# PixelClear/OclPathTracer

Measured on AMD Instinct MI355X. Metric: Msamples/sec (pixels x spp / s), cornellbox.bin 1024x1024, higher is better.
Workload: dtype f32; 1 GPU; BASELINE configs[2]: cornellbox.bin 1024x1024, 256 spp, depth 16, full path; render_lanes=2, checkpointed_launches=True, staging_ring_bytes=402653184, workspace_bytes=490036560

## Files before the change

### include/pt_shim.h

```cpp
#ifndef PT_SHIM_H
#define PT_SHIM_H

#include <stddef.h>
#include <stdint.h>

#ifdef __cplusplus
extern "C" {
#endif

#define PT_SHIM_ABI_VERSION 2

enum pt_status {
    PT_OK = 0,
    PT_ERR_INVALID = 1,
    PT_ERR_NO_DEVICE = 2,
    PT_ERR_OOM = 3,
    PT_ERR_HIP = 4,
    PT_ERR_NOT_FOUND = 5,
    PT_ERR_ARGS = 6,
    PT_ERR_RANGE = 7,
    PT_ERR_TRAVERSAL = 8
};

typedef struct pt_device_s* pt_device_t;
typedef struct pt_buffer_s* pt_buffer_t;
typedef struct pt_kernel_s* pt_kernel_t;
typedef struct pt_event_s* pt_event_t;

const char* pt_last_error(void);
int pt_abi_version(void);

int pt_init(void);
void pt_quit(void);
int pt_device_count(void);
int pt_device_create(int device_idx, pt_device_t* out);
int pt_device_destroy(pt_device_t dev);

enum pt_info_kind {
    PT_INFO_NAME = 0,
    PT_INFO_BOARD = 1,
    PT_INFO_VENDOR = 2,
    PT_INFO_VERSION = 3
};
int pt_device_info(pt_device_t dev, int kind, char out[128]);
uint64_t pt_device_max_alloc(pt_device_t dev);
uint64_t pt_device_mem_size(pt_device_t dev);
uint64_t pt_device_used_memory(pt_device_t dev);
uint64_t pt_device_peak_memory(pt_device_t dev);
uint64_t pt_device_workspace_memory(pt_device_t dev);
int pt_device_reserve_staging(pt_device_t dev, size_t bytes);
int pt_device_num_cus(pt_device_t dev);

#define PT_STREAM_LEGACY ((void*)1)
int pt_device_set_stream(pt_device_t dev, void* hip_stream);
void* pt_device_get_stream(pt_device_t dev);
int pt_device_wait_stream(pt_device_t dev, void* hip_stream);
int pt_device_wait_hip_event(pt_device_t dev, void* hip_event);
int pt_event_wait_on(pt_event_t ev, void* hip_stream);

int pt_sync(pt_device_t dev);
int pt_flush(pt_device_t dev);

enum pt_option {
    PT_OPT_BATCH_FRAMES = 0,
    PT_OPT_CHUNK_FRAMES = 1,
    PT_OPT_PROFILE_RETURN_TIME = 2,
    PT_OPT_RESERVED_3 = 3,
    PT_OPT_QUAD_FILTER = 4,
    PT_OPT_ACCEL = 5,
    PT_OPT_BVH_TALLY = 6,
    PT_OPT_PRIMARY_MASKS = 7,
    PT_OPT_BVH_STACK_LIMIT = 8,
    PT_OPT_RENDER_LANES = 9,
    PT_OPT_CHECKPOINT = 10,
    PT_OPT_BVH_BUILD_COUNT = 11
};
int pt_device_set_option(pt_device_t dev, int option, int64_t value);
int64_t pt_device_get_option(pt_device_t dev, int option);

int pt_buffer_alloc(pt_device_t dev, size_t bytes, pt_buffer_t* out);
int pt_buffer_wrap(pt_device_t dev, void* device_ptr, size_t bytes, pt_buffer_t* out);
int pt_buffer_free(pt_buffer_t buf);
size_t pt_buffer_size(pt_buffer_t buf);
void* pt_buffer_device_ptr(pt_buffer_t buf);
void* pt_buffer_address(pt_buffer_t buf);
int pt_buffer_write(pt_buffer_t dst, const void* host_src, size_t bytes, size_t dst_offset, pt_event_t ev);
int pt_buffer_read(pt_buffer_t src, void* host_dst, size_t bytes, size_t src_offset, pt_event_t ev);
int pt_buffer_copy(pt_buffer_t dst, pt_buffer_t src, size_t bytes, size_t dst_offset, size_t src_offset, pt_event_t ev);
void* pt_buffer_map(pt_buffer_t buf, size_t bytes, int blocking);
int pt_buffer_unmap(pt_buffer_t buf, void* host_ptr);

int pt_host_alloc(size_t bytes, void** out);
int pt_host_free(void* host_ptr);

int pt_event_create(pt_device_t dev, pt_event_t* out);
int pt_event_destroy(pt_event_t ev);
int pt_event_wait(pt_event_t ev);
int pt_event_is_complete(pt_event_t ev);
int pt_event_elapsed_ns(pt_event_t ev, uint64_t* ns_out);

int pt_kernel_get(pt_device_t dev, const char* file_name, const char* func_name, pt_kernel_t* out);

#define PT_MAX_ARG_SIZE 64
#define PT_MAX_ARG_COUNT 64

typedef struct pt_launch_arg {
    int32_t is_buffer;
    int32_t read_only;
    uint64_t size;
    pt_buffer_t buffer;
    unsigned char data[PT_MAX_ARG_SIZE];
} pt_launch_arg;

int pt_launch_2d(pt_device_t dev, pt_kernel_t kernel, const pt_launch_arg* args, int nargs,
                 int num_threads_x, int num_threads_y, int local_x, int local_y,
                 pt_event_t ev, float* ms_out);

typedef struct pt_render_params {
    int32_t width, height;
    int32_t frame_begin;
    int32_t frame_count;
    int32_t max_bounces;
    int32_t num_triangles;
    int32_t num_materials;
    int32_t stripe_rows;
    int32_t n_ranks;
    int32_t rank;
    int32_t reserved[6];
} pt_render_params;

int pt_local_rows(int height, int stripe_rows, int n_ranks, int rank);

enum {
    PT_STAT_SAMPLES = 0, PT_STAT_RAYS = 1,
    PT_STAT_BVH_NODES = 2, PT_STAT_BVH_TRIS = 3, PT_STAT_BVH_STEPS = 4 , PT_STAT_BVH_TRI_STEPS = 5,
    PT_STAT_BVH_MAX_STACK = 6 ,
    PT_STAT_CARRIED = 7 ,
    PT_STAT_BVH_GRAZING = 8,
    PT_STAT_WORDS = 16
};

int pt_render_frames(pt_device_t dev, pt_buffer_t triangles, pt_buffer_t materials,
                     pt_buffer_t framebuffer, const pt_render_params* params,
                     pt_buffer_t stats ,
                     pt_event_t ev);

typedef struct pt_camera {
    float eye[3];
    float center[3];
    float up[3];
    float fov_y_deg;
    int32_t reserved[6];
} pt_camera;

void pt_camera_reference(pt_camera* out);
int pt_camera_derive(const pt_camera* cam, float out[16]);
int pt_render_frames_camera(pt_device_t dev, pt_buffer_t triangles, pt_buffer_t materials, pt_buffer_t framebuffer,
                            const pt_render_params* params, const pt_camera* cam,
// ... 102 lines not shown
                       pt_buffer_t noise , pt_buffer_t summary , pt_event_t ev);

typedef struct pt_adaptive_rule {
    double tol2;
    double floor2;
    uint32_t min_samples;
    uint32_t max_samples;
    uint32_t reserved[2];
} pt_adaptive_rule;
typedef struct pt_pixel_slot { uint32_t pixel; uint32_t frame; } pt_pixel_slot;
size_t pt_adaptive_list_bytes(uint32_t num_pixels);
int pt_adaptive_select(pt_device_t dev, pt_buffer_t moments , uint32_t num_pixels,
                       const pt_adaptive_rule* rule, pt_buffer_t list , pt_event_t ev);
int pt_render_indirect_pixels(pt_device_t dev, pt_buffer_t triangles, pt_buffer_t materials,
                              pt_buffer_t lights , int mis,
                              pt_buffer_t light_counts ,
                              pt_buffer_t cdf, pt_buffer_t tri_q , pt_buffer_t samples ,
                              pt_buffer_t framebuffer, pt_buffer_t list, uint32_t num_listed, const pt_indirect_params* params,
                              const pt_roulette* roulette, const pt_camera* cam , pt_event_t ev);
int pt_sample_moments_pixels(pt_device_t dev, pt_buffer_t samples ,
                             pt_buffer_t moments , pt_buffer_t list, uint32_t num_listed, int32_t frame_count,
                             pt_event_t ev);

typedef struct pt_ris {
    int32_t candidates;
    int32_t reserved[3];
} pt_ris;
int pt_render_direct_ris(pt_device_t dev, pt_buffer_t triangles, pt_buffer_t materials,
                         pt_buffer_t lights , pt_buffer_t cdf, pt_buffer_t tri_q ,
                         pt_buffer_t samples , pt_buffer_t framebuffer, const pt_direct_params* params, const pt_ris* ris,
                         const pt_camera* cam , pt_event_t ev);
int pt_render_indirect_ris(pt_device_t dev, pt_buffer_t triangles, pt_buffer_t materials,
                           pt_buffer_t lights , int mis,
                           pt_buffer_t light_counts ,
                           pt_buffer_t cdf, pt_buffer_t tri_q , pt_buffer_t samples ,
                           pt_buffer_t framebuffer, const pt_indirect_params* params, const pt_roulette* roulette, const pt_ris* ris,
                           const pt_camera* cam , pt_event_t ev);
int pt_render_indirect_pixels_ris(pt_device_t dev, pt_buffer_t triangles, pt_buffer_t materials,
                                  pt_buffer_t lights , int mis,
                                  pt_buffer_t light_counts ,
                                  pt_buffer_t cdf, pt_buffer_t tri_q , pt_buffer_t samples ,
                                  pt_buffer_t framebuffer, pt_buffer_t list, uint32_t num_listed, const pt_indirect_params* params,
                                  const pt_roulette* roulette, const pt_ris* ris, const pt_camera* cam ,
                                  pt_event_t ev);

typedef struct pt_environment {
    int32_t size;
    int32_t env_samples;
    int32_t reserved[2];
} pt_environment;
size_t pt_env_table_bytes(int size);
int pt_env_table(pt_device_t dev, pt_buffer_t env , int size, pt_buffer_t cdf ,
                 pt_event_t ev);
int pt_render_direct_env(pt_device_t dev, pt_buffer_t triangles, pt_buffer_t materials,
                         pt_buffer_t lights , pt_buffer_t cdf, pt_buffer_t tri_q ,
                         pt_buffer_t env, pt_buffer_t env_cdf , pt_buffer_t samples ,
                         pt_buffer_t framebuffer, const pt_direct_params* params, const pt_environment* environment,
                         const pt_camera* cam , pt_event_t ev);
int pt_render_indirect_env(pt_device_t dev, pt_buffer_t triangles, pt_buffer_t materials,
                           pt_buffer_t lights ,
                           pt_buffer_t light_counts, pt_buffer_t cdf, pt_buffer_t tri_q ,
                           pt_buffer_t env, pt_buffer_t env_cdf , pt_buffer_t samples ,
                           pt_buffer_t framebuffer, const pt_indirect_params* params, const pt_roulette* roulette,
                           const pt_environment* environment, const pt_camera* cam , pt_event_t ev);

enum { PT_PROF_TRACE = 0, PT_PROF_FOLD = 1, PT_PROF_KINDS = 2 };
int pt_profile_enable(pt_device_t dev, int on);
int pt_profile_query(pt_device_t dev, int kind, double* total_ms, uint64_t* launches);
int pt_profile_query_union(pt_device_t dev, int kind, double* union_ms);
int pt_profile_reset(pt_device_t dev);

#define PT_BVH_SNAPSHOT_BIG_MAX 64
typedef struct pt_bvh_info {
    uint32_t records;
    int32_t num_big;
    int32_t num_triangles;
    float grid_min[3], grid_step[3];
    int32_t reserved[7];
} pt_bvh_info;
int pt_bvh_snapshot(pt_device_t dev, pt_bvh_info* info, void* records, size_t record_capacity, int32_t* big_indices);

int pt_primary_mask_snapshot(pt_device_t dev, uint32_t* num_pixels, void* masks, size_t capacity);

int pt_assemble_stripes(pt_device_t dev, pt_buffer_t gathered, pt_buffer_t image, int width,
                        int height, int stripe_rows, int n_ranks, int slab_rows, pt_event_t ev);

int pt_assemble_stripes_on(pt_device_t dev, pt_buffer_t gathered, pt_buffer_t image, int width, int height,
                           int stripe_rows, int n_ranks, int slab_rows, void* hip_stream);

int pt_tonemap_ppm(pt_device_t dev, pt_buffer_t framebuffer, pt_buffer_t rgb_i32, size_t num_pixels,
                   pt_event_t ev);

#ifdef __cplusplus
}
#endif
#endif
```

### oclpathtracer_amd/csrc/pt_kernels.h

```cpp
#pragma once

#include <hip/hip_runtime.h>
#include <stdint.h>

struct PtRawTriangle { float p1[4], p2[4], p3[4]; int32_t id; char pad[12]; };
struct PtRawMaterial { float albedo[4], emissive[4]; float roughness; int32_t type; char pad[24]; };
static_assert(sizeof(PtRawTriangle) == 64 && sizeof(PtRawMaterial) == 64, "record layout");

struct PtPrepTriangle {
    float p1[3];
    float e1[3];
    float e2[3];
    float pad0[3];
    float n[3];
    int32_t id;
};
static_assert(sizeof(PtPrepTriangle) == 64, "prep layout");

struct PtBvhNode {
    float lmin[3]; uint32_t link_l;
    float lmax[3]; uint32_t link_r;
    float rmin[3]; uint32_t pad0;
    float rmax[3]; uint32_t pad1;
};
static_assert(sizeof(PtBvhNode) == 64, "bvh node layout");

struct alignas(64) PtBvh8Node {
    uint16_t org[3];
    uint8_t ex[3];
    uint8_t imask;
    uint8_t lmask;
    uint8_t pad;
    uint32_t base;
    uint8_t qlo[3][8];
    uint8_t qhi[3][8];
};
static_assert(sizeof(PtBvh8Node) == 64, "bvh node layout");
struct PtBvhGrid { float gmin[3], gstep[3]; };

struct alignas(64) PtLeafTri {
    float p1[3], e1[3], e2[3];
    uint32_t index;
    float pad[6];
};
static_assert(sizeof(PtLeafTri) == 64, "leaf record layout");

#define PT_TRACE_BATCH 256u
#define PT_TRACE_THREADS 256
#define PT_LDS_TRI_STRIDE 12
#define PT_LDS_TRI_MAX 256

struct PtCamera {
    float eye[3], view[3], hol[3], up[3];
    float angle;
};

struct PtTraceParams {
    const PtPrepTriangle* tris;
    const PtRawMaterial* mats;
    float* rad;
    float* rad1;
    unsigned int* batch_counter;
    unsigned long long* stats;
    int32_t width, height;
    float inv_width, inv_height, aspect;
    int32_t frame_begin;
    int32_t frame_count;
    uint32_t chunk_f0;
    uint32_t slot_frames;
    uint32_t ring_phase;
    uint32_t ring_magic;
    uint32_t rad1_off;
    int32_t max_bounces, ntri, nmat;
    int32_t stripe_rows, n_ranks, rank;
    uint32_t npix_local;
    uint32_t batches_per_frame, total_batches;
    uint32_t batch;
    float quad_delta1;
    float ray_radius;
    const float* p1tab;
    float p1_lo, p1_hi;
    const PtBvh8Node* bvh;
    int32_t bvh_records;
    PtBvhGrid grid;
    const PtPrepTriangle* bigtab;
    const int32_t* bigidx;
    int32_t nbig;
    const uint2* pmask;
    unsigned int* bvh_flags;
    int32_t bvh_stack_limit;
    uint32_t* carry;
    uint32_t carry_in_waves;
    uint32_t carry_out;
    PtCamera cam;
};
#define PT_QUEUE_SHARDS 8
#define PT_QUEUE_SHARD_WORDS 1056
#define PT_QUEUE_STOP_WORD (PT_QUEUE_SHARDS * PT_QUEUE_SHARD_WORDS)
#define PT_QUEUE_WORDS ((PT_QUEUE_SHARDS + 1) * PT_QUEUE_SHARD_WORDS)
#define PT_CARRY_RECORDS 64
#define PT_CARRY_STRIDE_DW (16 + PT_CARRY_RECORDS * 15)
#define PT_CARRY_HIT_STRIDE_DW (16 + PT_CARRY_RECORDS * 18)
#define PT_PACKED_BOUNCE_MAX 256

struct PtFoldParams {
    const float* rad;
    float4* fb;
    uint32_t npix_local;
    int32_t frame_begin, frame_count;
    unsigned int* reset_counter;
    unsigned int* reset_counter2;
};

#define PT_PREP_WORDS 12
__host__ __device__ static inline unsigned ptk_order_key(float f)
{
    unsigned u;
    __builtin_memcpy(&u, &f, sizeof u);
    return (u & 0x80000000u) ? ~u : (u | 0x80000000u);
}
__host__ __device__ static inline float ptk_order_float(unsigned k)
{
    const unsigned u = (k & 0x80000000u) ? (k & 0x7fffffffu) : ~k;
    float f;
    __builtin_memcpy(&f, &u, sizeof f);
    return f;
}
hipError_t ptk_prep_triangles(const PtRawTriangle* raw, PtPrepTriangle* out, int ntri, unsigned int* det_bound_bits,
                              hipStream_t s);
hipError_t ptk_prep_quad_margins(PtPrepTriangle* out, int ntri, float diameter, float delta1, float* p1tab, const float anchor[3], hipStream_t s);
#define PT_P1_STRIDE 24
static inline size_t ptk_p1tab_floats(int ntri) { return (size_t)((ntri / 2 + 1) / 2) * PT_P1_STRIDE; }
hipError_t ptk_primary_masks(const PtTraceParams& p, hipStream_t s);
struct PtSearchMode {
    bool bvh;
    bool det_bounded;
    int quads;
};
hipError_t ptk_trace(const PtTraceParams& p, int num_blocks, PtSearchMode m, bool tally, bool wide, hipStream_t s);
#define PT_BVH_NEAR_EYE 4.0f
hipError_t ptk_bvh_big_raw(const PtRawTriangle* raw, const int* bigidx, int nbig, PtRawTriangle* out, hipStream_t s);
static inline size_t ptk_bvh_record_count(int ntri) { return 2 * (size_t)(ntri > 0 ? ntri : 0); }
size_t ptk_bvh_temp_bytes(int ntri);
#define PT_BVH_BIG_MAX 64
#define PT_BVH_RAY_EPS 1.2e-4f
hipError_t ptk_bvh_build(const PtRawTriangle* raw, const PtPrepTriangle* prep, int ntri, PtBvh8Node* recs,
                         PtPrepTriangle* bigtab, int* bigidx, int* nbig_dev, PtBvhGrid* grid_dev, unsigned* used_dev, void* temp, size_t temp_bytes,
                         hipStream_t s);
#define PT_DET_BOUND_MAX 2.0e19f
#define PT_BVH_AUTO_MIN 512
hipError_t ptk_fold(const PtFoldParams& p, hipStream_t s);
hipError_t ptk_assemble_stripes(const float4* gathered, float4* image, int width, int height, int stripe_rows,
                                int n_ranks, int slab_rows, hipStream_t s);
hipError_t ptk_tonemap_ppm(const float4* fb, int32_t* rgb, size_t npix, hipStream_t s);
hipError_t ptk_fill_i32(int32_t* dst, int32_t value, int n, hipStream_t s);
hipError_t ptk_math(const float* in, float* out, int n, hipStream_t s);
hipError_t ptk_fold_check(unsigned long long* out, int mode, unsigned first, unsigned long long count, hipStream_t s);
hipError_t ptk_shade_check(unsigned long long* out, int mode, unsigned first, unsigned long long count, hipStream_t s);
struct PtQueryParams {
    PtTraceParams t;
    const float4* rays;
    void* out;
    uint32_t nrays;
    int32_t occluded;
};
hipError_t ptk_query(const PtQueryParams& q, int bvh_blocks, PtSearchMode m, bool any, hipStream_t s);
int ptk_query_bvh_blocks_per_cu(void);
struct PtAoParams {
    PtTraceParams t;
    PtCamera cam;
    unsigned long long* counts;
    uint32_t npix;
    uint32_t nitems;
    int32_t frame0;
    int32_t K;
    float tlim;
};
hipError_t ptk_ao(const PtAoParams& a, int bvh_blocks, PtSearchMode m, hipStream_t s);
hipError_t ptk_ao_resolve(const uint2* counts, float4* image, uint32_t npix, uint32_t K, float miss_value, hipStream_t s);
struct PtDirectParams {
    PtTraceParams t;
    PtCamera cam;
    const int32_t* lights;
    float* samples;
    uint32_t npix;
    uint32_t nitems;
    int32_t frame0;
    int32_t K;
    int32_t nl;
};
struct PtIndirectParams {
    PtDirectParams d;
    int32_t B;
};
struct PtIndirectMisParams : PtIndirectParams {
    const int32_t* counts;
};
hipError_t ptk_light_counts(const int32_t* lights, int nl, int ntri, int32_t* counts, hipStream_t s);
struct PtDirectPowerParams : PtDirectParams {
    const uint64_t* cdf;
    const uint32_t* tri_q;
};
struct PtIndirectPowerParams : PtIndirectMisParams {
    const uint64_t* cdf;
    const uint32_t* tri_q;
};
struct PtIndirectRrParams : PtIndirectPowerParams {
    int32_t R;
    float cap;
};
struct PtIndirectListParams : PtIndirectRrParams {
    const uint2* slots;
    uint32_t frame_off;
};
struct PtDirectRisParams : PtDirectPowerParams {
    int32_t M;
// ... 79 lines not shown
```

### oclpathtracer_amd/csrc/pt_kernels.hip

```cpp
#include "pt_kernels.h"

#include "pt_device_math.h"

#include <type_traits>

typedef const __attribute__((address_space(4))) float* pt_const_f32p;

PTK_DEV unsigned pt_lane_id() { return __builtin_amdgcn_mbcnt_hi(~0u, __builtin_amdgcn_mbcnt_lo(~0u, 0u)); }
PTK_DEV unsigned pt_mbcnt(unsigned long long m) { return __builtin_amdgcn_mbcnt_hi((unsigned)(m >> 32), __builtin_amdgcn_mbcnt_lo((unsigned)m, 0u)); }

typedef const __attribute__((address_space(4))) PtTraceParams* pt_kargs_p;
PTK_DEV pt_kargs_p pt_kargs()
{
    pt_kargs_p k = (pt_kargs_p)__builtin_amdgcn_kernarg_segment_ptr();
    asm volatile("" : "+s"(k));
    return k;
}
PTK_DEV f3 pt_anchor()
{
    const pt_kargs_p K = pt_kargs();
    return mk3(K->cam.eye[0], K->cam.eye[1], K->cam.eye[2]);
}
#define PT_ARG(field) (LATE ? K->field : P.field)

__global__ void pt_prep_kernel(const PtRawTriangle* __restrict__ raw, PtPrepTriangle* __restrict__ out, int ntri,
                               unsigned int* __restrict__ det_bound_bits)
{
    int i = blockIdx.x * blockDim.x + threadIdx.x;
    if (i >= ntri) return;
    f3 p1 = mk3(raw[i].p1[0], raw[i].p1[1], raw[i].p1[2]);
    f3 p2 = mk3(raw[i].p2[0], raw[i].p2[1], raw[i].p2[2]);
    f3 p3 = mk3(raw[i].p3[0], raw[i].p3[1], raw[i].p3[2]);
    f3 e1 = sub3(p2, p1);
    f3 e2 = sub3(p3, p1);
    f3 n = cross3(e2, e1);
    PtPrepTriangle t;
    t.p1[0] = p1.x; t.p1[1] = p1.y; t.p1[2] = p1.z;
    t.e1[0] = e1.x; t.e1[1] = e1.y; t.e1[2] = e1.z;
    t.e2[0] = e2.x; t.e2[1] = e2.y; t.e2[2] = e2.z;
    t.pad0[0] = t.pad0[1] = t.pad0[2] = 0.0f;
    t.n[0] = n.x; t.n[1] = n.y; t.n[2] = n.z;
    t.id = raw[i].id;
    out[i] = t;
    float b = (__builtin_fabsf(e1.x) + __builtin_fabsf(e1.y) + __builtin_fabsf(e1.z)) *
              (__builtin_fabsf(e2.x) + __builtin_fabsf(e2.y) + __builtin_fabsf(e2.z));
    atomicMax(&det_bound_bits[0], __float_as_uint(b) & 0x7fffffffu);
    if (i & 1) {
        f3 q1 = mk3(raw[i - 1].p1[0], raw[i - 1].p1[1], raw[i - 1].p1[2]);
        f3 q3 = mk3(raw[i - 1].p3[0], raw[i - 1].p3[1], raw[i - 1].p3[2]);
        f3 f2 = sub3(q3, q1);
        if (!(e2.x == -f2.x && e2.y == -f2.y && e2.z == -f2.z)) atomicAdd(&det_bound_bits[1], 1u);
        if (!(p1.x == q3.x && p1.y == q3.y && p1.z == q3.z)) atomicAdd(&det_bound_bits[3], 1u);
    }
    {
        const f3 vs[3] = { p1, p2, p3 };
        bool fin = true;
        float lo[3], hi[3];
        for (int a = 0; a < 3; ++a) { lo[a] = hi[a] = a == 0 ? p1.x : a == 1 ? p1.y : p1.z; }
        for (int k = 0; k < 3; ++k) {
            const float c[3] = { vs[k].x, vs[k].y, vs[k].z };
            for (int a = 0; a < 3; ++a) {
                fin = fin && __builtin_isfinite(c[a]);
                lo[a] = c[a] < lo[a] ? c[a] : lo[a];
                hi[a] = c[a] > hi[a] ? c[a] : hi[a];
            }
        }
        if (!fin) atomicOr(&det_bound_bits[2], 1u);
        for (int a = 0; a < 3; ++a) {
            atomicMax(&det_bound_bits[6 + a], ~ptk_order_key(lo[a]));
            atomicMax(&det_bound_bits[9 + a], ptk_order_key(hi[a]));
        }
    }
    {
        const unsigned* w = reinterpret_cast<const unsigned*>(raw + i);
        unsigned long long h = 0x9e3779b97f4a7c15ull * (unsigned long long)(i + 1);
        for (int k = 0; k < 16; ++k) {
            h ^= (unsigned long long)w[k] + 0x9e3779b97f4a7c15ull + (h << 6) + (h >> 2);
            h *= 0xff51afd7ed558ccdull;
            h ^= h >> 33;
        }
        atomicAdd(reinterpret_cast<unsigned long long*>(det_bound_bits + 4), h);
    }
}

__global__ void pt_prep_quad_margins_kernel(PtPrepTriangle* __restrict__ out, int ntri, float diameter, float delta1)
// ... 51 lines not shown
    x = (2.0f * ((x + 0.5f) * inv_w) - 1.0f) * angle * aspect;
    y = -(1.0f - 2.0f * ((y + 0.5f) * inv_h)) * angle;

    float my = -1.0f * y;
    f3 d = add3(add3(scale3(holDir, x), scale3(upDir, my)), viewDir);
    f3 dir = normalize3(d);
    f3 pointAimed = add3(eye, scale3(dir, 4.0f));
    org = eye;
    aim = normalize3(sub3(pointAimed, eye));
}

PTK_DEV void pt_camera_ray(float x, float y, float inv_w, float inv_h, float aspect, const PtCam& c, f3& org, f3& dir_out)
{
    f3 aim;
    pt_camera_aim(x, y, inv_w, inv_h, aspect, c, org, aim);
    dir_out = normalize3(aim);
}

PTK_DEV void pt_pixel_jitter(int xc, int yc, uint32_t& seed, float& x, float& y)
{
    x = (float)xc + pt_random_float(seed) - 0.5f;
    y = (float)yc + pt_random_float(seed) - 0.5f;
}

PTK_DEV void pt_generate_ray(int xc, int yc, float inv_w, float inv_h, float aspect, const PtCam& c, uint32_t& seed, f3& org, f3& dir_out)
{
    float x, y;
    pt_pixel_jitter(xc, yc, seed, x, y);
    pt_camera_ray(x, y, inv_w, inv_h, aspect, c, org, dir_out);
}

struct PtMaskParams {
    const PtPrepTriangle* tris;
    uint2* out;
    int32_t width, height, ntri;
    int32_t stripe_rows, n_ranks, rank;
    uint32_t npix_local;
    PtCamera cam;
};

PTK_DEV float pt_norm1(const f3& a) { return __builtin_fabsf(a.x) + __builtin_fabsf(a.y) + __builtin_fabsf(a.z); }

__global__ void pt_primary_mask_kernel(const PtMaskParams P)
{
    const unsigned lp = blockIdx.x * blockDim.x + threadIdx.x;
    if (lp >= P.npix_local) return;
    const unsigned lr = lp / (unsigned)P.width, x = lp - lr * (unsigned)P.width;
    unsigned grow = lr;
    if (P.n_ranks > 1) {
        const unsigned sl = lr / (unsigned)P.stripe_rows;
        const unsigned within = lr - sl * (unsigned)P.stripe_rows;
        grow = (sl * (unsigned)P.n_ranks + (unsigned)P.rank) * (unsigned)P.stripe_rows + within;
    }
    f3 o, dc;
    const PtCam cam = PT_CAM_K(P.cam);
    pt_camera_ray((float)x, (float)grow, 1.0f / (float)P.width, 1.0f / (float)P.height, (float)P.width / (float)P.height, cam, o, dc);
    const float hx = cam.angle * ((float)P.width / (float)P.height) / (float)P.width;
    const float hy = cam.angle / (float)P.height;
    const float eps = __builtin_sqrtf(hx * hx + hy * hy) * 1.01f + 4e-6f;
    const float uS = (32.0f + 8.0f * eps) * 5.9604645e-8f;
    const float A = 2e-24f;
    unsigned m[2] = { 0u, 0u };
    for (int j = 0; j < P.ntri; ++j) {
        const PtPrepTriangle* t = P.tris + j;
        const f3 e1 = mk3(t->e1[0], t->e1[1], t->e1[2]), e2 = mk3(t->e2[0], t->e2[1], t->e2[2]);
        const f3 tv = mk3(o.x - t->p1[0], o.y - t->p1[1], o.z - t->p1[2]);
        const f3 Kd = cross3(e2, e1), Ku = cross3(e2, tv), qv = cross3(tv, e1);
        const float tn = dot3(e2, qv);
        const float detc = dot3(dc, Kd), unc = dot3(dc, Ku), vnc = dot3(dc, qv);
        const float a1 = pt_norm1(e1), a2 = pt_norm1(e2), at = pt_norm1(tv);
        const float rho_d = (eps * pt_norm1(Kd) + uS * (a1 * a2)) * 1.001f + A;
        const float rho_u = (eps * pt_norm1(Ku) + uS * (at * a2)) * 1.001f + A;
        const float rho_v = (eps * pt_norm1(qv) + uS * (at * a1)) * 1.001f + A;
        const bool keep = !(detc + rho_d < 0.999e-8f)
                        & !(unc + rho_u < 0.0f)
                        & !(vnc + rho_v < 0.0f)
                        & !((unc - rho_u) + (vnc - rho_v) > (detc + rho_d) * 1.000002f)
                        & !(tn <= 0.0f);
        const int c = j >> 5;
        const int nc = P.ntri - 32 * c < 32 ? P.ntri - 32 * c : 32;
        m[c] |= (keep ? 1u : 0u) << (nc - 1 - (j & 31));
    }
    P.out[lp] = make_uint2(m[0], m[1]);
}

struct PtTriRec { float p1x, p1y, p1z, e1x, e1y, e1z, e2x, e2y, e2z; };

PTK_DEV PtTriRec pt_load_tri(pt_const_f32p T, int i)
{
    pt_const_f32p t = T + 16 * i;
    PtTriRec r;
    r.p1x = t[0]; r.p1y = t[1]; r.p1z = t[2];
    r.e1x = t[3]; r.e1y = t[4]; r.e1z = t[5];
    r.e2x = t[6]; r.e2y = t[7]; r.e2z = t[8];
    return r;
}

#ifndef PT_VALIDATE_FILTER
#define PT_VALIDATE_FILTER 0
#endif
typedef unsigned long long pt_lanes;
#define PT_LANES(cond) __builtin_amdgcn_ballot_w64(cond)
#define PT_ON(mask) __builtin_amdgcn_inverse_ballot_w64(mask)
PTK_DEV unsigned pt_push_flag(unsigned m, pt_lanes c)
{
    unsigned long long carry_out;
    unsigned r;
    asm("v_addc_co_u32_e64 %0, %1, %2, %2, %3" : "=v"(r), "=s"(carry_out) : "v"(m), "s"(c));
    return r;
}

template <bool DET_BOUNDED>
PTK_DEV pt_lanes pt_tri_pass1(const PtTriRec& r, const f3& o, const f3& d)
{
    float pvx = pt_fma(d.y, r.e2z, -(d.z * r.e2y));
    float pvy = pt_fma(d.z, r.e2x, -(d.x * r.e2z));
    float pvz = pt_fma(d.x, r.e2y, -(d.y * r.e2x));
    float det = pt_fma(r.e1z, pvz, pt_fma(r.e1y, pvy, r.e1x * pvx));
    float tvx = o.x - r.p1x, tvy = o.y - r.p1y, tvz = o.z - r.p1z;
    float un = pt_fma(tvz, pvz, pt_fma(tvy, pvy, tvx * pvx));
    pt_lanes ok;
    if (DET_BOUNDED) {
        ok = PT_LANES(!(un < -1e-24f)) & PT_LANES(!(un > det * 1.000001f));
    } else {
        float u = un * (1.0f / det);
        ok = PT_LANES(!(det < 1e-8f)) & PT_LANES(!(u < 0.0f)) & PT_LANES(!(u > 1.0f));
    }
    return ok;
}

extern __shared__ __attribute__((aligned(16))) float pt_lds_tab[];

template <int LDS_TABLE>
PTK_DEV PtTriRec pt_fetch_rec(const PtPrepTriangle* tris, int i, unsigned lds_off = 0u)
{
    float4 q0, q1;
    float e2z;
    if (LDS_TABLE) {
        typedef __attribute__((address_space(3))) const float pt_lds_f32;
        typedef float pt_v4 __attribute__((ext_vector_type(4)));
        typedef __attribute__((address_space(3))) const pt_v4 pt_lds_f32x4;
        pt_lds_f32* t = (pt_lds_f32*)pt_lds_tab + lds_off + __umul24((unsigned)i, (unsigned)PT_LDS_TRI_STRIDE);
        const pt_v4 a = *(pt_lds_f32x4*)t, b = *(pt_lds_f32x4*)(t + 4);
        q0 = make_float4(a.x, a.y, a.z, a.w);
        q1 = make_float4(b.x, b.y, b.z, b.w);
        e2z = t[8];
    } else {
        const float* t = reinterpret_cast<const float*>(tris + i);
        q0 = *reinterpret_cast<const float4*>(t);
        q1 = *reinterpret_cast<const float4*>(t + 4);
        e2z = t[8];
    }
    PtTriRec r;
    r.p1x = q0.x; r.p1y = q0.y; r.p1z = q0.z;
    r.e1x = q0.w; r.e1y = q1.x; r.e1z = q1.y;
    r.e2x = q1.z; r.e2y = q1.w; r.e2z = e2z;
    return r;
}

PTK_DEV void pt_stage_tile(const PtPrepTriangle* tris, int base, int n, unsigned tile_off, unsigned lane)
{
    const float* g = reinterpret_cast<const float*>(tris + base);
    for (unsigned k = lane; k < (unsigned)n * PT_LDS_TRI_STRIDE; k += 64u) {
        const unsigned tri = k / PT_LDS_TRI_STRIDE, w = k - tri * PT_LDS_TRI_STRIDE;
        pt_lds_tab[tile_off + k] = g[tri * 16u + w];
    }
// ... 250 lines not shown
            pt_const_f32p tp = p1tab + PT_P1_STRIDE * (base >> 2);
            for (int j = 0; j < n; j += 4, tp += PT_P1_STRIDE) {
                pt_f2 un, th;
                pt_quad3_pass1(tp, r3v, un, th);
                {
                    const pt_lanes in = PT_LANES(!(__builtin_fabsf(un.x) > th.x));
                    m = pt_push_flag(pt_push_flag(m, in & PT_LANES(!(un.x < p1_lo))), in & PT_LANES(!(un.x > p1_hi)));
                }
                if (j + 2 < n) {
                    const pt_lanes in = PT_LANES(!(__builtin_fabsf(un.y) > th.y));
                    m = pt_push_flag(pt_push_flag(m, in & PT_LANES(!(un.y < p1_lo))), in & PT_LANES(!(un.y > p1_hi)));
                }
            }
            if (!tame) m = n == 32 ? ~0u : (1u << n) - 1u;
        } else {
            PtTriRec a = pt_load_tri(T, base);
            int j = 0;
            for (; j + 1 < n; j += 2) {
                PtTriRec b = pt_load_tri(T, base + j + 1);
                m = pt_push_flag(m, pt_tri_pass1<DET_BOUNDED>(a, o, d));
                a = pt_load_tri(T, base + (j + 2 < n ? j + 2 : j + 1));
                m = pt_push_flag(m, pt_tri_pass1<DET_BOUNDED>(b, o, d));
            }
            if (j < n) m = pt_push_flag(m, pt_tri_pass1<DET_BOUNDED>(a, o, d));
        }
#if PT_VALIDATE_FILTER
        if (alive && vstat) {
            unsigned mx = 0u;
            for (int jj = 0; jj < n; ++jj) {
                const PtTriRec r = pt_load_tri(T, base + jj);
                float pvx = pt_fma(d.y, r.e2z, -(d.z * r.e2y));
                float pvy = pt_fma(d.z, r.e2x, -(d.x * r.e2z));
                float pvz = pt_fma(d.x, r.e2y, -(d.y * r.e2x));
                float det = pt_fma(r.e1z, pvz, pt_fma(r.e1y, pvy, r.e1x * pvx));
                bool keep = !(det < 1e-8f || -det > 1e-8f);
                float inv_det = 1.0f / det;
                float tvx = o.x - r.p1x, tvy = o.y - r.p1y, tvz = o.z - r.p1z;
                float u = pt_fma(tvz, pvz, pt_fma(tvy, pvy, tvx * pvx)) * inv_det;
                keep = keep && !(u < 0.0f || u > 1.0f);
                mx |= (keep ? 1u : 0u) << (n - 1 - jj);
            }
            atomicAdd(&vstat[0], (unsigned long long)n);
            atomicAdd(&vstat[1], (unsigned long long)__popc(mx));
            atomicAdd(&vstat[2], (unsigned long long)__popc(m));
            atomicAdd(&vstat[3], (unsigned long long)__popc(mx & ~m));
            if (QUADS == 3 && DET_BOUNDED && tame) {
                float r1 = 0.0f, r3 = 0.0f;
                {
                    const float deltaP = -p1_lo, deltaD = deltaP * (128.0f / 192.0f);
                    for (int jj = 0; jj + 1 < n; jj += 4) {
                        pt_f2 unp, thp;
                        pt_const_f32p tq = p1tab + PT_P1_STRIDE * ((base + jj) >> 2);
                        pt_quad3_pass1(tq, r3v, unp, thp);
                        for (int h = 0; h < 2 && jj + 2 * h + 1 < n; ++h) {
                            const PtTriRec a = pt_load_tri(T, base + jj + 2 * h);
                            float pvx = pt_fma(d.y, a.e2z, -(d.z * a.e2y)), pvy = pt_fma(d.z, a.e2x, -(d.x * a.e2z)), pvz = pt_fma(d.x, a.e2y, -(d.y * a.e2x));
                            float detA = pt_fma(a.e1z, pvz, pt_fma(a.e1y, pvy, a.e1x * pvx));
                            float unA = pt_fma(o.z - a.p1z, pvz, pt_fma(o.y - a.p1y, pvy, (o.x - a.p1x) * pvx));
                            const float dhi = tq[18 + h];
                            const float q1 = __builtin_fabsf((h ? unp.y : unp.x) - unA) / deltaP;
                            const float q3 = __builtin_fabsf(((h ? thp.y : thp.x) - dhi) - detA * 1.000002f) / deltaD;
                            r1 = q1 > r1 ? q1 : r1;
                            r3 = q3 > r3 ? q3 : r3;
                        }
                    }
                }
                atomicMax(&vstat[4], (unsigned long long)__float_as_uint(r1));
                atomicMax(&vstat[5], (unsigned long long)__float_as_uint(r3));
            }
        }
#endif
        if (!alive) m = 0u;
#if PT_STAMPS
        PT_STAMP(tb);
        if (p1_ticks) *p1_ticks += tb - ta;
#endif
        pt_pass2_chunk<DET_BOUNDED, LDS_TABLE>(m, base, n, tris, o, d, tmax, hu, hv, hidx, tl, lane, steps);
    }
    pt_pass2_finish<DET_BOUNDED, LDS_TABLE>(tris, o, d, tmax, hu, hv, hidx, tl, lane, steps);
    return steps;
}

template <bool DET_BOUNDED, int LDS_TABLE>
PTK_DEV unsigned pt_intersect_primary(pt_const_f32p T, const PtPrepTriangle* tris, int ntri, const f3& o, const f3& d, bool alive,
                                      float& tmax, float& hu, float& hv, int& hidx, uint2 pm, PtTail tl, unsigned lane,
                                      unsigned long long* vstat = nullptr)
{
    (void)T; (void)vstat;
    tl.wr = tl.rd = 0u;
    tl.kbest = ~0ull;
    unsigned steps = 0;
    for (int base = 0; base < ntri; base += 32) {
        const int n = ntri - base < 32 ? ntri - base : 32;
        unsigned m = base == 0 ? pm.x : pm.y;
#if PT_VALIDATE_FILTER
        if (alive && vstat) {
            unsigned mx = 0u;
            for (int jj = 0; jj < n; ++jj) {
                const PtTriRec r = pt_load_tri(T, base + jj);
                float pvx = pt_fma(d.y, r.e2z, -(d.z * r.e2y));
                float pvy = pt_fma(d.z, r.e2x, -(d.x * r.e2z));
                float pvz = pt_fma(d.x, r.e2y, -(d.y * r.e2x));
                float det = pt_fma(r.e1z, pvz, pt_fma(r.e1y, pvy, r.e1x * pvx));
                bool keep = !(det < 1e-8f || -det > 1e-8f);
                float inv_det = 1.0f / det;
                float tvx = o.x - r.p1x, tvy = o.y - r.p1y, tvz = o.z - r.p1z;
                float u = pt_fma(tvz, pvz, pt_fma(tvy, pvy, tvx * pvx)) * inv_det;
                keep = keep && !(u < 0.0f || u > 1.0f);
                float qvx = pt_fma(tvy, r.e1z, -(tvz * r.e1y));
                float qvy = pt_fma(tvz, r.e1x, -(tvx * r.e1z));
                float qvz = pt_fma(tvx, r.e1y, -(tvy * r.e1x));
                float v = pt_fma(d.z, qvz, pt_fma(d.y, qvy, d.x * qvx)) * inv_det;
                keep = keep && !(v < 0.0f || u + v > 1.0f);
                float tt = pt_fma(r.e2z, qvz, pt_fma(r.e2y, qvy, r.e2x * qvx)) * inv_det;
                keep = keep && (tt > 0.0f && tt < 1e20f);
                mx |= (keep ? 1u : 0u) << (n - 1 - jj);
            }
            atomicAdd(&vstat[0], (unsigned long long)n);
            atomicAdd(&vstat[1], (unsigned long long)__popc(mx));
            atomicAdd(&vstat[2], (unsigned long long)__popc(m));
            atomicAdd(&vstat[3], (unsigned long long)__popc(mx & ~m));
        }
#endif
        if (!alive) m = 0u;
        pt_pass2_chunk<DET_BOUNDED, LDS_TABLE>(m, base, n, tris, o, d, tmax, hu, hv, hidx, tl, lane, steps);
    }
    pt_pass2_finish<DET_BOUNDED, LDS_TABLE>(tris, o, d, tmax, hu, hv, hidx, tl, lane, steps);
    return steps;
}


struct PtPath {
    f3 o, d;
    f3 mask, L;
    uint32_t seed;
    int bounce;
    unsigned ro;
    unsigned fl;
};

PTK_DEV unsigned pt_ring_offset(unsigned lp, unsigned frame)
{
    const pt_kargs_p KR = pt_kargs();
    const unsigned fr = frame + KR->ring_phase, S = KR->slot_frames;
    const unsigned r = fr - __umulhi(fr, KR->ring_magic) * (2u * S);
    const bool upper = r >= S;
    return (upper ? KR->rad1_off : 0u) + ((upper ? r - S : r) * KR->npix_local + lp) * 12u;
}



PTK_DEV void pt_shade_miss(PtPath& s)
{
    const float bg = pt_max(0.45f, 0.0f);
    s.L = add3(s.L, scale3(s.mask, bg));
}

template <bool DET_BOUNDED, bool LATE>
PTK_DEV bool pt_shade_hit(const PtTraceParams& P, PtPath& s, const f3 p, float hu, float hv, int hidx)
{
    const pt_kargs_p K = pt_kargs();
    bool finished = false;
    {
        float phi = PTK_TWO_PI * pt_random_float(s.seed);
        float xi = pt_random_float(s.seed);
        float sp, cp;
        __builtin_amdgcn_sched_barrier(0);
// ... 428 lines not shown
    s.seed = gid + pt_hash_u32((uint32_t)f);
    pt_generate_ray((int)x, (int)grow, PT_ARG(inv_width), PT_ARG(inv_height), PT_ARG(aspect), PT_CAM_K(K->cam), s.seed, s.o, s.d);
    s.mask = mk3(1.0f, 1.0f, 1.0f);
    s.L = mk3(0.0f, 0.0f, 0.0f);
    s.bounce = 0;
    s.ro = K->rad1_off != 0u ? pt_ring_offset(lp, frame) : lp;
    s.fl = frame;
}

template <bool LATE>
PTK_DEV bool pt_start_fresh(const PtTraceParams& P, unsigned lane, PtWaveQueue& q, PtPath& s, pt_lanes& alive, unsigned& pix0)
{
    const pt_kargs_p K = pt_kargs();
    pix0 = q.pix;
    const unsigned avail = q.end - q.pix;
    const unsigned count = avail < 64u ? avail : 64u;
    const unsigned W = (unsigned)PT_ARG(width), SR = (unsigned)PT_ARG(stripe_rows);
    if (lane < count) {
        unsigned x = q.col + lane, up = 0u;
        while (x >= W) { x -= W; ++up; }
        unsigned grow = q.row + up;
        if (PT_ARG(n_ranks) > 1) {
            unsigned sl = q.sl, within = q.within + up;
            while (within >= SR) { within -= SR; ++sl; }
            grow = pt_stripe_row<LATE>(P, K, sl, within);
        }
        pt_sample_begin<LATE>(P, K, x, grow, q.pix + lane, q.frame, s);
    }
    alive = count == 64u ? ~0ull : (1ull << count) - 1ull;
    q.pix += count;
    q.col += count;
    while (q.col >= W) {
        q.col -= W;
        ++q.row;
        if (++q.within == SR) { q.within = 0u; ++q.sl; }
    }
    return count == 64u;
}

PTK_DEV PtPath pt_path_idle()
{
    PtPath s;
    s.o = mk3(0.0f, 0.0f, 0.0f); s.d = mk3(0.0f, 0.0f, 1.0f);
    s.mask = mk3(1.0f, 1.0f, 1.0f); s.L = mk3(0.0f, 0.0f, 0.0f);
    s.seed = 0; s.bounce = 0; s.ro = 0; s.fl = 0;
    return s;
}

PTK_DEV unsigned pt_wave_in_wg() { return (unsigned)__builtin_amdgcn_readfirstlane(threadIdx.x >> 6); }
PTK_DEV unsigned pt_wave() { return blockIdx.x * (PT_TRACE_THREADS / 64) + pt_wave_in_wg(); }
PTK_DEV uint32_t* pt_carry_region(uint32_t* carry, unsigned wave, unsigned stride = PT_CARRY_STRIDE_DW) { return carry + (size_t)wave * stride; }

PTK_DEV PtTail pt_tail_init(pt_lds_u32* w, unsigned tile, unsigned lane)
{
    PtTail tl;
    tl.keys = (pt_lds_u64*)w;
    tl.list = w + 128;
    tl.wr = tl.rd = 0u;
    tl.kbest = ~0ull; tl.ku = tl.kv = 0.0f;
    tl.tile = tile;
    tl.keys[lane] = ~0ull;
    return tl;
}

PTK_DEV void pt_lds_table_load(const PtPrepTriangle* tris, int n)
{
    const float* g = reinterpret_cast<const float*>(tris);
    for (int k = (int)threadIdx.x; k < n * PT_LDS_TRI_STRIDE; k += PT_TRACE_THREADS) {
        const int tri = k / PT_LDS_TRI_STRIDE, w = k - tri * PT_LDS_TRI_STRIDE;
        pt_lds_tab[k] = g[tri * 16 + w];
    }
}

#define PT_LDS_TILE_DW (32u * PT_LDS_TRI_STRIDE)
template <int LDS_TABLE> __host__ __device__ __forceinline__ unsigned pt_lds_tail_dw() { return 128u + (LDS_TABLE == 1 ? PT_TAIL_LIST / 2u : PT_TAIL_LIST); }
template <int LDS_TABLE> __host__ __device__ __forceinline__ unsigned pt_lds_pools(int ntri) { return LDS_TABLE == 1 ? ntri * PT_LDS_TRI_STRIDE : 0; }
template <int LDS_TABLE, bool POOLS = true> __host__ __device__ __forceinline__ unsigned pt_lds_tails(int ntri) { return pt_lds_pools<LDS_TABLE>(ntri) + (POOLS ? (PT_TRACE_THREADS / 64) * pt_pool_dwords<LDS_TABLE>() : 0u); }
template <int LDS_TABLE, bool POOLS = true> __host__ __device__ __forceinline__ unsigned pt_lds_tiles(int ntri) { return pt_lds_tails<LDS_TABLE, POOLS>(ntri) + (PT_TRACE_THREADS / 64) * pt_lds_tail_dw<LDS_TABLE>(); }
template <int LDS_TABLE, bool POOLS = true> __host__ __device__ __forceinline__ unsigned pt_lds_total(int ntri) { return pt_lds_tiles<LDS_TABLE, POOLS>(ntri) + (LDS_TABLE == 2 ? (PT_TRACE_THREADS / 64) * PT_LDS_TILE_DW : 0u); }

#ifndef PT_TRACE_UNIT_DIR
#define PT_TRACE_UNIT_DIR 1
#endif
template <bool DET_BOUNDED, int LDS_TABLE, int QUADS>
PTK_DEV void pt_trace_body(const PtTraceParams& P)
{
    const unsigned lane = pt_lane_id();
    pt_const_f32p T = (pt_const_f32p)(const float*)P.tris;
    const int ntri = P.ntri;
    if (LDS_TABLE == 1) {
        pt_lds_table_load(P.tris, ntri);
        __syncthreads();
    }
    const unsigned wave_in_wg = pt_wave_in_wg();
    constexpr unsigned NW = pt_hit_words<LDS_TABLE>();
    float4* pool = reinterpret_cast<float4*>(pt_lds_tab + pt_lds_pools<LDS_TABLE>(ntri) + wave_in_wg * pt_pool_dwords<LDS_TABLE>());
    unsigned pool_n = 0u;
    PtTail tl = pt_tail_init((pt_lds_u32*)pt_lds_tab + pt_lds_tails<LDS_TABLE>(ntri) + (threadIdx.x >> 6) * pt_lds_tail_dw<LDS_TABLE>(),
                             pt_lds_tiles<LDS_TABLE>(ntri) + (threadIdx.x >> 6) * PT_LDS_TILE_DW, lane);

    PtWaveQueue q = { 0u, 0u, 0u, 0u, 0u, 0u, 0u, 0u };
    pt_lanes alive = 0ull;
    PtPath s = pt_path_idle();
    PtHit h = { 0.0f, 0.0f, -1 };
    pt_lanes ended = 0ull;
    unsigned n_rays = 0, n_samples = 0, n_carried = 0;
    const unsigned wave = pt_wave();
    if (wave < P.carry_in_waves) {
        bool resumed = false;
        pt_carry_hit_load<true, NW>(P, pt_carry_region(P.carry, wave, PT_CARRY_HIT_STRIDE_DW), lane, s, h, resumed, q, n_rays, n_samples, n_carried);
        alive = PT_LANES(resumed);
    }
    q.g = wave & (PT_QUEUE_SHARDS - 1u);
#if PT_STAMPS
    unsigned long long t0 = 0, t1 = 0, t2 = 0, t3 = 0, c_regen = 0, c_loop = 0, c_shade = 0, c_iters = 0, c_steps = 0, c_p1 = 0;
#endif

    for (;;) {
        PT_STAMP(t0);
        {
            const pt_lanes missed = alive & PT_LANES(h.hidx < 0);
            if (PT_ON(missed)) pt_shade_miss(s);
            const pt_lanes over = missed | ended;
            if (PT_ON(over)) pt_path_finish(s);
            n_samples += (unsigned)__popcll(over);
            alive &= ~missed;
            ended = 0ull;
        }
        bool fresh = false;
        bool primary = false;
        unsigned pix0 = 0u;
        if (~alive != 0ull) {
            if (pool_n == 0u && (unsigned)__popcll(alive) <= (unsigned)PT_POOL) {
                const int next = pt_queue_next<true>(P, lane, q, s, alive);
                if (next != 0) {
                    pt_pool_push<NW>(pool, pool_n, s, h, alive);
                    if (next == 2) break;
                    primary = pt_start_fresh<true>(P, lane, q, s, alive, pix0);
                    fresh = true;
                }
            }
            if (!fresh) pt_pool_pop<NW>(pool, pool_n, s, h, alive);
        }
        if (!fresh && alive == 0ull) break;
        PT_STAMP(t1);

        if (!fresh) {
            bool finished = false;
            if (PT_ON(alive)) finished = pt_shade_hit<DET_BOUNDED, true>(P, s, s.o, h.hu, h.hv, h.hidx);
            ended = PT_LANES(finished);
            alive &= ~ended;
        }
        PT_STAMP(t2);

        float tmax = 1e20f, hu = 0.0f, hv = 0.0f;
        int hidx = -1;
        unsigned p2steps = 0;
        n_rays += (unsigned)__popcll(alive);
        if (alive == 0ull) {
        } else if (QUADS == 3 && DET_BOUNDED && primary && P.pmask != nullptr)
            p2steps = pt_intersect_primary<DET_BOUNDED, LDS_TABLE>(T, P.tris, ntri, s.o, s.d, PT_ON(alive), tmax, hu, hv, hidx, P.pmask[pix0 + lane], tl, lane,
                                                                   PT_VALIDATE_FILTER && P.stats ? P.stats + 2 : nullptr);
        else
            p2steps = pt_intersect_two_pass<DET_BOUNDED, LDS_TABLE, QUADS, PT_TRACE_UNIT_DIR != 0>(T, P.tris, ntri, s.o, s.d, PT_ON(alive), tmax, hu, hv, hidx,
                                                                                          P.quad_delta1, P.ray_radius,
                                                                                          (pt_const_f32p)P.p1tab, P.p1_lo, P.p1_hi, pt_anchor(), tl, lane,
                                                                                          PT_VALIDATE_FILTER && P.stats ? P.stats + 2 : nullptr,
#if PT_STAMPS
                                                                                          &c_p1
#else
                                                                                          nullptr
#endif
                                                                                          );
#if PT_STAMPS
        c_steps += p2steps;
#else
        (void)p2steps;
#endif

        s.o = add3(s.o, scale3(s.d, tmax));
        h.hu = hu; h.hv = hv; h.hidx = hidx;
#if PT_STAMPS
        PT_STAMP(t3);
        c_regen += t1 - t0; c_shade += t2 - t1; c_loop += t3 - t2; c_iters++;
#endif
    }

#if PT_STAMPS
    if (P.stats && lane == 0) {
        atomicAdd(&P.stats[2], c_regen);
        atomicAdd(&P.stats[3], c_loop);
        atomicAdd(&P.stats[4], c_shade);
        atomicAdd(&P.stats[5], c_iters);
        atomicAdd(&P.stats[7], c_steps);
        atomicAdd(&P.stats[6], c_p1);
    }
#endif
    {
        const pt_kargs_p K = pt_kargs();
        if (K->carry_out != 0u) {
            pt_carry_store<NW>(pt_carry_region(K->carry, wave, PT_CARRY_HIT_STRIDE_DW), lane, pool, pool_n, q, n_rays, n_samples, n_carried);
            return;
        }
    }
#if !PT_STAMPS && !PT_VALIDATE_FILTER
    if (P.stats && lane == 0 && n_carried != 0u) atomicAdd(&P.stats[7], (unsigned long long)n_carried);
#endif
    pt_flush_counters(P, lane, n_rays, n_samples);
}

#ifndef PT_TRACE_WAVES
#define PT_TRACE_WAVES 8
#endif
template <bool DET_BOUNDED, int LDS_TABLE, int QUADS>
__global__ __launch_bounds__(PT_TRACE_THREADS) __attribute__((amdgpu_waves_per_eu(PT_TRACE_WAVES, PT_TRACE_WAVES)))
void pt_trace_kernel(const PtTraceParams P)
{
    pt_trace_body<DET_BOUNDED, LDS_TABLE, QUADS>(P);
}

template <bool DET_BOUNDED>
__global__ __launch_bounds__(PT_TRACE_THREADS) __attribute__((amdgpu_waves_per_eu(6, 6)))
void pt_trace_tiled_kernel(const PtTraceParams P)
{
    pt_trace_body<DET_BOUNDED, 2, 0>(P);
}

#ifndef PT_BVH_STACK
#define PT_BVH_STACK 64
#endif
#ifndef PT_BVH_LDS_STACK
#define PT_BVH_LDS_STACK 8
#endif
#ifndef PT_BVH_REFILL
#define PT_BVH_REFILL 40
#endif

#define PT_BVH_TAIL_DW (128u + PT_TAIL_LIST)
__host__ __device__ __forceinline__ unsigned pt_bvh_lds_stacks() { return PT_BVH_BIG_MAX * PT_LDS_TRI_STRIDE; }
__host__ __device__ __forceinline__ unsigned pt_bvh_lds_tails() { return pt_bvh_lds_stacks() + 2 * PT_BVH_LDS_STACK * PT_TRACE_THREADS; }
__host__ __device__ __forceinline__ unsigned pt_bvh_lds_nxt() { return pt_bvh_lds_tails() + (PT_TRACE_THREADS / 64) * PT_BVH_TAIL_DW; }
__host__ __device__ __forceinline__ unsigned pt_bvh_lds_total() { return pt_bvh_lds_nxt() + 2048u / 4u; }

template <bool LATE>
PTK_DEV void pt_regenerate_lanes(const PtTraceParams& P, unsigned lane, PtWaveQueue& q, PtPath& s, bool& alive)
// ... 2410 lines not shown

__global__ __launch_bounds__(PT_LIGHT_SCAN_BLOCK) void pt_adaptive_scatter_kernel(const PtPixelMoments* __restrict__ moments, uint32_t npix,
                                                                                  const PtAdaptiveRule R, const uint64_t* __restrict__ tile_sums,
                                                                                  uint2* __restrict__ slots)
{
    __shared__ uint64_t lds[PT_LIGHT_SCAN_BLOCK];
    const uint64_t first = (uint64_t)blockIdx.x * PT_LIGHT_SCAN_TILE + threadIdx.x * PT_LIGHT_SCAN_ITEMS;
    uint32_t frame[PT_LIGHT_SCAN_ITEMS];
    unsigned active = 0u;
    for (unsigned k = 0; k < PT_LIGHT_SCAN_ITEMS; ++k) {
        uint64_t taken = 0ull;
        if (first + k < (uint64_t)npix && pt_adaptive_active(moments[first + k], R, &taken)) active |= 1u << k;
        frame[k] = (uint32_t)taken;
    }
    uint64_t total;
    uint64_t at = tile_sums[blockIdx.x] + pt_light_block_scan((uint64_t)__popc(active), lds, &total);
    for (unsigned k = 0; k < PT_LIGHT_SCAN_ITEMS; ++k)
        if (active & (1u << k)) slots[at++] = make_uint2((uint32_t)(first + k), frame[k]);
}

hipError_t ptk_fold_list(const PtFoldListParams& p, hipStream_t s)
{
    if (p.num_listed == 0 || p.frame_count <= 0) return hipSuccess;
    hipLaunchKernelGGL(pt_fold_list_kernel, dim3((unsigned)(((size_t)p.num_listed * 3 + 255) / 256)), dim3(256), 0, s, p);
    return hipGetLastError();
}

hipError_t ptk_sample_moments_list(const float* samples, PtPixelMoments* moments, const uint2* slots, uint32_t num_listed, uint32_t npix,
                                   int32_t frames, hipStream_t s)
{
    if (num_listed == 0 || npix == 0 || frames <= 0) return hipSuccess;
    hipLaunchKernelGGL(pt_sample_moments_list_kernel, dim3((unsigned)(((uint64_t)num_listed + 255u) / 256u)), dim3(256), 0, s, samples, moments, slots,
                       num_listed, npix, frames);
    return hipGetLastError();
}

hipError_t ptk_adaptive_select(const PtPixelMoments* moments, uint32_t npix, const PtAdaptiveRule& rule, void* list, hipStream_t s)
{
    if (npix == 0) return hipMemsetAsync(list, 0, 16, s);
    const unsigned ntiles = (unsigned)PT_LIGHT_TABLE_TILES(npix);
    uint2* slots = reinterpret_cast<uint2*>(static_cast<char*>(list) + 16);
    uint64_t* tile_sums = reinterpret_cast<uint64_t*>(slots + npix);
    hipLaunchKernelGGL(pt_adaptive_count_kernel, dim3(ntiles), dim3(PT_LIGHT_SCAN_BLOCK), 0, s, moments, npix, rule, tile_sums);
    hipLaunchKernelGGL(pt_adaptive_tiles_kernel, dim3(1), dim3(PT_LIGHT_SCAN_BLOCK), 0, s, tile_sums, ntiles, static_cast<uint32_t*>(list));
    hipLaunchKernelGGL(pt_adaptive_scatter_kernel, dim3(ntiles), dim3(PT_LIGHT_SCAN_BLOCK), 0, s, moments, npix, rule, tile_sums, slots);
    return hipGetLastError();
}

hipError_t ptk_prep_triangles(const PtRawTriangle* raw, PtPrepTriangle* out, int ntri, unsigned int* det_bound_bits,
                              hipStream_t s)
{
    hipError_t e = hipMemsetAsync(det_bound_bits, 0, PT_PREP_WORDS * sizeof(unsigned int), s);
    if (e != hipSuccess || ntri <= 0) return e;
    hipLaunchKernelGGL(pt_prep_kernel, dim3((ntri + 255) / 256), dim3(256), 0, s, raw, out, ntri, det_bound_bits);
    return hipGetLastError();
}

hipError_t ptk_prep_quad_margins(PtPrepTriangle* out, int ntri, float diameter, float delta1, float* p1tab, const float anchor[3], hipStream_t s)
{
    if (ntri < 2) return hipSuccess;
    const int pairs = ntri / 2;
    hipLaunchKernelGGL(pt_prep_quad_margins_kernel, dim3((pairs + 255) / 256), dim3(256), 0, s, out, ntri, diameter, delta1);
    if (p1tab) {
        const int qpairs = (pairs + 1) / 2;
        hipLaunchKernelGGL(pt_prep_p1tab_kernel, dim3((qpairs + 255) / 256), dim3(256), 0, s, out, ntri, diameter, p1tab, anchor[0], anchor[1], anchor[2]);
    }
    return hipGetLastError();
}

hipError_t ptk_primary_masks(const PtTraceParams& p, hipStream_t s)
{
    if (!p.pmask || p.npix_local == 0) return hipSuccess;
    PtMaskParams m;
    m.tris = p.tris;
    m.out = const_cast<uint2*>(p.pmask);
    m.width = p.width; m.height = p.height; m.ntri = p.ntri;
    m.stripe_rows = p.stripe_rows; m.n_ranks = p.n_ranks; m.rank = p.rank;
    m.npix_local = p.npix_local;
    m.cam = p.cam;
    hipLaunchKernelGGL(pt_primary_mask_kernel, dim3((p.npix_local + 255u) / 256u), dim3(256), 0, s, m);
    return hipGetLastError();
}

hipError_t ptk_trace(const PtTraceParams& p, int num_blocks, PtSearchMode m, bool tally, bool wide, hipStream_t s)
{
    const bool q3 = m.quads == 3;
    void (*kernel)(const PtTraceParams);
    if (m.bvh && wide)
        kernel = tally ? (m.det_bounded ? (q3 ? pt_trace_bvh_kernel<true, true, 3, true> : pt_trace_bvh_kernel<true, true, 0, true>) : pt_trace_bvh_kernel<false, true, 0, true>)
                       : (m.det_bounded ? (q3 ? pt_trace_bvh_kernel<true, false, 3, true> : pt_trace_bvh_kernel<true, false, 0, true>) : pt_trace_bvh_kernel<false, false, 0, true>);
    else if (m.bvh)
        kernel = tally ? (m.det_bounded ? (q3 ? pt_trace_bvh_kernel<true, true, 3> : pt_trace_bvh_kernel<true, true, 0>) : pt_trace_bvh_kernel<false, true, 0>)
                       : (m.det_bounded ? (q3 ? pt_trace_bvh_kernel<true, false, 3> : pt_trace_bvh_kernel<true, false, 0>) : pt_trace_bvh_kernel<false, false, 0>);
    else if (p.ntri <= PT_LDS_TRI_MAX)
        kernel = m.det_bounded ? (q3 ? pt_trace_kernel<true, 1, 3> : pt_trace_kernel<true, 1, 0>) : pt_trace_kernel<false, 1, 0>;
    else
        kernel = m.det_bounded ? pt_trace_tiled_kernel<true> : pt_trace_tiled_kernel<false>;
    const size_t lds = m.bvh ? ptk_trace_bvh_lds_bytes() : ptk_trace_lds_bytes(p.ntri);
    hipLaunchKernelGGL(kernel, dim3(num_blocks), dim3(PT_TRACE_THREADS), lds, s, p);
    return hipGetLastError();
}

hipError_t ptk_fold(const PtFoldParams& p, hipStream_t s)
{
    if (p.npix_local == 0) return hipSuccess;
    hipLaunchKernelGGL(pt_fold_kernel, dim3((unsigned)(((size_t)p.npix_local * 3 + 255) / 256)), dim3(256), 0, s, p);
    return hipGetLastError();
}

hipError_t ptk_assemble_stripes(const float4* gathered, float4* image, int width, int height, int stripe_rows,
                                int n_ranks, int slab_rows, hipStream_t s)
{
    size_t total = (size_t)width * height;
    if (total == 0) return hipSuccess;
    hipLaunchKernelGGL(pt_assemble_kernel, dim3((unsigned)((total + 255) / 256)), dim3(256), 0, s, gathered, image,
                       width, height, stripe_rows, n_ranks, slab_rows);
    return hipGetLastError();
}

hipError_t ptk_tonemap_ppm(const float4* fb, int32_t* rgb, size_t npix, hipStream_t s)
{
    if (npix == 0) return hipSuccess;
    hipLaunchKernelGGL(pt_tonemap_kernel, dim3((unsigned)((npix + 255) / 256)), dim3(256), 0, s, fb, rgb, npix);
    return hipGetLastError();
}

hipError_t ptk_fold_check(unsigned long long* out, int mode, unsigned first, unsigned long long count, hipStream_t s)
{
    if (count == 0) return hipSuccess;
    const unsigned long long want = (count + 255) / 256;
    hipLaunchKernelGGL(pt_fold_check_kernel, dim3((unsigned)(want < 65536ull ? want : 65536ull)), dim3(256), 0, s, out, mode, first, count);
    return hipGetLastError();
}

hipError_t ptk_shade_check(unsigned long long* out, int mode, unsigned first, unsigned long long count, hipStream_t s)
{
    if (count == 0) return hipSuccess;
    const unsigned long long want = (count + 255) / 256;
    hipLaunchKernelGGL(pt_shade_check_kernel, dim3((unsigned)(want < 65536ull ? want : 65536ull)), dim3(256), 0, s, out, mode, first, count);
    return hipGetLastError();
}

hipError_t ptk_math(const float* in, float* out, int n, hipStream_t s)
{
    if (n <= 0) return hipSuccess;
    hipLaunchKernelGGL(pt_math_kernel, dim3((n + 255) / 256), dim3(256), 0, s, in, out, n);
    return hipGetLastError();
}

hipError_t ptk_fill_i32(int32_t* dst, int32_t value, int n, hipStream_t s)
{
    if (n <= 0) return hipSuccess;
    hipLaunchKernelGGL(pt_fill_i32_kernel, dim3((n + 255) / 256), dim3(256), 0, s, dst, value, n);
    return hipGetLastError();
}

size_t ptk_trace_lds_bytes(int ntri)
{
    return (size_t)(ntri <= PT_LDS_TRI_MAX ? pt_lds_total<1>(ntri) : pt_lds_total<2>(ntri)) * sizeof(float);
}

size_t ptk_trace_bvh_lds_bytes(void)
{
    return (size_t)pt_bvh_lds_total() * sizeof(float);
}

// ... 218 lines not shown
```

### oclpathtracer_amd/csrc/pt_shim.hip

```cpp
#include "../../include/pt_shim.h"

#include <hip/hip_runtime.h>

#include <algorithm>
#include <cmath>
#include <cstdarg>
#include <cstdio>
#include <cstdlib>
#include <cstring>
#include <initializer_list>
#include <new>
#include <string>
#include <utility>
#include <vector>

#include "pt_kernels.h"

static thread_local char g_err[512] = "";

static int fail(int code, const char* fmt, ...)
{
    va_list ap;
    va_start(ap, fmt);
    vsnprintf(g_err, sizeof g_err, fmt, ap);
    va_end(ap);
    return code;
}

#define HIP_TRY(expr)                                                                          \
    do {                                                                                       \
        hipError_t e_ = (expr);                                                                \
        if (e_ != hipSuccess) return fail(PT_ERR_HIP, "%s failed: %s", #expr, hipGetErrorString(e_)); \
    } while (0)

extern "C" const char* pt_last_error(void) { return g_err; }
extern "C" int pt_abi_version(void) { return PT_SHIM_ABI_VERSION; }

enum { KERNEL_GENERATE_COLORS = 0, KERNEL_FILL = 1, KERNEL_MATH = 2, KERNEL_FOLD_CHECK = 3, KERNEL_SHADE_CHECK = 4, KERNEL_COUNT = 5 };

struct pt_kernel_s {
    int id;
    const char* file;
    const char* func;
};

struct pt_buffer_s {
    pt_device_s* dev;
    void* dptr;
    size_t bytes;
    bool owned;
    uint64_t version;
    void* staging;
    size_t staging_bytes;
    bool mapped;
    size_t mapped_bytes;
    bool exposed;
};

struct pt_event_s {
    pt_device_s* dev;
    hipEvent_t start, stop;
    bool recorded;
};

struct PendingFrames {
    bool active;
    pt_buffer_s *tris, *mats, *fb;
    int width, height, z_begin, z_count;
    uint32_t pixel_count;
};

template <class T> struct PtWs {
    T* p;
    size_t bytes;
    operator T*() const { return p; }
};

struct PtFilterTable {
    bool pairs;
    int quads;
    float anchor[3]; bool anchor_valid;
    PtWs<float> p1tab;
    float delta1, ray_radius, p1_lo, p1_hi;
};

struct pt_device_s {
    int idx;
    hipDeviceProp_t prop;
    hipStream_t own_stream, stream;
    bool external;
    uint64_t used, peak;
    int live_buffers;
    uint64_t workspace;
    int64_t opt_batch, opt_chunk, opt_profile, opt_quads, opt_accel, opt_tally, opt_pmask, opt_bvh_stack, opt_lanes, opt_carry;
    pt_kernel_s kernels[KERNEL_COUNT];
    PendingFrames pending;
    PtWs<PtPrepTriangle> prep;
    size_t prep_capacity;
    const pt_buffer_s* prep_src;
    uint64_t prep_version;
    int prep_ntri;
    uint64_t prep_hash;
    bool prep_hash_valid;
    uint64_t scene_gen;
    bool prep_det_bounded;
    bool prep_finite;
    float prep_lo[3], prep_hi[3];
    PtWs<unsigned int> det_bound_dev;
    int blocks_per_cu;
    PtFilterTable scene_filter;
    PtFilterTable big_filter;
    PtWs<PtBvh8Node> bvh;
    PtBvhGrid bvh_grid;
    size_t bvh_records;
    PtWs<PtPrepTriangle> bigtab;
    PtWs<int> bigidx;
    int nbig;
    bool bvh_valid;
    uint64_t bvh_builds;
    int bvh_blocks_per_cu;
    int query_bvh_blocks_per_cu;
    int lit_bvh_blocks_per_cu[PT_LIT_KIND_INDICES];
    unsigned int* trav_host;
    unsigned int* trav_dev;
    PtWs<float> ring;
    size_t ring_slot_bytes;
    hipStream_t lane[2];
    hipEvent_t ev_fork;
    hipEvent_t ev_fold[2];
    hipEvent_t ev_slot[2];
    hipEvent_t ev_ext;
    bool fold_recorded[2], slot_recorded[2];
    int last_fold_lane;
    bool lanes_busy;
    bool main_dirty;
    uint64_t chunk_seq, render_seq;
    PtWs<uint32_t> carry[2];
    PtWs<uint2> pmask;
    struct { uint64_t scene_gen; int32_t g[7]; PtCamera cam; bool valid; } pmask_key;
    PtWs<unsigned int> counters;
    bool counters_dirty;
    bool prof_on;
    std::vector<std::pair<hipEvent_t, hipEvent_t>> prof_pairs[PT_PROF_KINDS];
    size_t prof_used[PT_PROF_KINDS];
};

#define PT_RING_SLOTS 2
#define PT_DEFAULT_SLOT_BYTES ((size_t)192 << 20)
#define PT_QUEUE_COUNTERS 64
#define PT_QUEUE_STRIDE PT_QUEUE_WORDS

static int prof_begin(pt_device_s* d, int kind, hipStream_t st, hipEvent_t* stop_out)
{
    *stop_out = nullptr;
    if (!d->prof_on) return PT_OK;
    auto& v = d->prof_pairs[kind];
    if (d->prof_used[kind] == v.size()) {
        hipEvent_t a, b;
        HIP_TRY(hipEventCreate(&a));
        HIP_TRY(hipEventCreate(&b));
        v.push_back({ a, b });
    }
    auto& pr = v[d->prof_used[kind]++];
    HIP_TRY(hipEventRecord(pr.first, st));
    *stop_out = pr.second;
    return PT_OK;
}

static int prof_end(hipStream_t st, hipEvent_t stop)
{
    if (stop) HIP_TRY(hipEventRecord(stop, st));
    return PT_OK;
}

#ifndef PT_DEFAULT_PRIMARY_MASKS
#define PT_DEFAULT_PRIMARY_MASKS 1
#endif

static int g_init_count = 0;

template <class T> static hipError_t ws_malloc(pt_device_s* d, PtWs<T>& w, size_t bytes)
{
    hipError_t e = hipMalloc(reinterpret_cast<void**>(&w.p), bytes);
    if (e == hipSuccess) { w.bytes = bytes; d->workspace += bytes; }
    else { w = {}; (void)hipGetLastError(); }
    return e;
}

template <class T> static void ws_free(pt_device_s* d, PtWs<T>& w)
{
    if (!w.p) return;
    hipFree(w.p);
    d->workspace -= w.bytes;
    w = {};
}

static const size_t WS_BIGTAB = PT_BVH_BIG_MAX * sizeof(PtPrepTriangle);
static const size_t WS_BIGIDX = (PT_BVH_BIG_MAX + 1) * sizeof(int) + sizeof(PtBvhGrid) + sizeof(unsigned);
static const size_t WS_COUNTERS = (size_t)PT_QUEUE_COUNTERS * PT_QUEUE_STRIDE * sizeof(unsigned int);
static const size_t WS_DETBOUND = PT_PREP_WORDS * sizeof(unsigned int);
static size_t ws_big_p1tab() { return ptk_p1tab_floats(PT_BVH_BIG_MAX) * sizeof(float) + PT_BVH_BIG_MAX * sizeof(PtRawTriangle); }

static int use_device(pt_device_s* d)
{
    if (!d) return fail(PT_ERR_INVALID, "null device handle");
    HIP_TRY(hipSetDevice(d->idx));
    return PT_OK;
}

extern "C" int pt_init(void)
{
    int n = 0;
    hipError_t e = hipGetDeviceCount(&n);
    if (e != hipSuccess) return fail(PT_ERR_NO_DEVICE, "hipGetDeviceCount: %s", hipGetErrorString(e));
    if (n <= 0) return fail(PT_ERR_NO_DEVICE, "no HIP device visible");
    ++g_init_count;
    return PT_OK;
}

extern "C" void pt_quit(void)
{
    if (g_init_count > 0) --g_init_count;
}

extern "C" int pt_device_count(void)
{
    int n = 0;
    if (hipGetDeviceCount(&n) != hipSuccess) return 0;
    return n;
}

static void destroy_device_objects(pt_device_s* d)
{
    ws_free(d, d->prep);
    ws_free(d, d->scene_filter.p1tab);
    ws_free(d, d->bvh);
    ws_free(d, d->ring);
    ws_free(d, d->pmask);
    ws_free(d, d->counters);
    ws_free(d, d->bigtab);
    ws_free(d, d->bigidx);
    ws_free(d, d->big_filter.p1tab);
    ws_free(d, d->det_bound_dev);
    if (d->trav_host) hipHostFree(d->trav_host);
    for (auto& v : d->prof_pairs)
        for (auto& pr : v) {
            hipEventDestroy(pr.first);
            hipEventDestroy(pr.second);
        }
    for (int k = 0; k < 2; ++k) {
        if (d->ev_fold[k]) hipEventDestroy(d->ev_fold[k]);
        if (d->ev_slot[k]) hipEventDestroy(d->ev_slot[k]);
        ws_free(d, d->carry[k]);
        if (d->lane[k]) hipStreamDestroy(d->lane[k]);
    }
    if (d->ev_fork) hipEventDestroy(d->ev_fork);
    if (d->ev_ext) hipEventDestroy(d->ev_ext);
    if (d->own_stream) hipStreamDestroy(d->own_stream);
    delete d;
}

extern "C" int pt_device_create(int device_idx, pt_device_t* out)
{
    if (!out) return fail(PT_ERR_INVALID, "out == NULL");
    *out = nullptr;
    int n = 0;
    hipError_t e = hipGetDeviceCount(&n);
    if (e != hipSuccess || n <= 0) return fail(PT_ERR_NO_DEVICE, "no HIP device visible (%s)", hipGetErrorString(e));
    if (device_idx < 0 || device_idx >= n) return fail(PT_ERR_NO_DEVICE, "device index %d out of range [0,%d)", device_idx, n);
    pt_device_s* d = new (std::nothrow) pt_device_s();
    if (!d) return fail(PT_ERR_OOM, "host allocation failed");
    d->idx = device_idx;
    if (hipSetDevice(device_idx) != hipSuccess || hipGetDeviceProperties(&d->prop, device_idx) != hipSuccess) {
        delete d;
        return fail(PT_ERR_HIP, "cannot open device %d", device_idx);
    }
    if (strncmp(d->prop.gcnArchName, "gfx950", 6) != 0) {
        char arch[64];
        snprintf(arch, sizeof arch, "%s", d->prop.gcnArchName);
        delete d;
        return fail(PT_ERR_NO_DEVICE, "device %d is %s; this library carries gfx950 (MI355X) code only", device_idx, arch);
    }
    if (hipStreamCreateWithFlags(&d->own_stream, hipStreamNonBlocking) != hipSuccess) {
        delete d;
        return fail(PT_ERR_HIP, "hipStreamCreate failed");
    }
    d->stream = d->own_stream;
    d->opt_batch = 1;
    d->opt_pmask = PT_DEFAULT_PRIMARY_MASKS;
    d->opt_bvh_stack = 64;
    d->opt_lanes = 2;
    d->opt_carry = 1;
    d->kernels[KERNEL_GENERATE_COLORS] = { KERNEL_GENERATE_COLORS, "GenerateColors", "GenerateColors" };
    d->kernels[KERNEL_FILL] = { KERNEL_FILL, "PtShimTest", "FillKernel" };
    d->kernels[KERNEL_MATH] = { KERNEL_MATH, "PtShimTest", "MathKernel" };
    d->kernels[KERNEL_FOLD_CHECK] = { KERNEL_FOLD_CHECK, "PtShimTest", "FoldCheckKernel" };
    d->kernels[KERNEL_SHADE_CHECK] = { KERNEL_SHADE_CHECK, "PtShimTest", "ShadeCheckKernel" };
    bool ok = ws_malloc(d, d->bigtab, WS_BIGTAB) == hipSuccess && ws_malloc(d, d->bigidx, WS_BIGIDX) == hipSuccess &&
              ws_malloc(d, d->counters, WS_COUNTERS) == hipSuccess && ws_malloc(d, d->big_filter.p1tab, ws_big_p1tab()) == hipSuccess &&
              ws_malloc(d, d->det_bound_dev, WS_DETBOUND) == hipSuccess;
    for (int k = 0; ok && k < 2; ++k)
        ok = hipStreamCreateWithFlags(&d->lane[k], hipStreamNonBlocking) == hipSuccess &&
             hipEventCreateWithFlags(&d->ev_fold[k], hipEventDisableTiming) == hipSuccess &&
             hipEventCreateWithFlags(&d->ev_slot[k], hipEventDisableTiming) == hipSuccess;
    ok = ok && hipEventCreateWithFlags(&d->ev_fork, hipEventDisableTiming) == hipSuccess &&
         hipEventCreateWithFlags(&d->ev_ext, hipEventDisableTiming) == hipSuccess;
    ok = ok && hipHostMalloc(reinterpret_cast<void**>(&d->trav_host), 64, hipHostMallocMapped) == hipSuccess &&
         hipHostGetDevicePointer(reinterpret_cast<void**>(&d->trav_dev), d->trav_host, 0) == hipSuccess;
    if (ok) {
        d->trav_host[0] = d->trav_host[1] = 0u;
        ok = hipMemsetAsync(d->counters, 0, WS_COUNTERS, d->own_stream) == hipSuccess && hipStreamSynchronize(d->own_stream) == hipSuccess;
    }
    if (!ok) {
        (void)hipGetLastError();
        destroy_device_objects(d);
        return fail(PT_ERR_OOM, "workspace allocation failed");
    }
    d->blocks_per_cu = ptk_trace_blocks_per_cu(36);
    d->bvh_blocks_per_cu = ptk_trace_bvh_blocks_per_cu();
    d->query_bvh_blocks_per_cu = ptk_query_bvh_blocks_per_cu();
    for (int i = 0; i < PT_LIT_KIND_INDICES; ++i) {
        const PtLitKind k = { (i & 1) != 0, (i & 2) != 0, (i & 4) != 0, (i & 8) != 0, (i & 16) != 0, (i & 32) != 0, (i & 64) != 0 };
        if (ptk_lit_kind_valid(k)) d->lit_bvh_blocks_per_cu[ptk_lit_kind_index(k)] = ptk_lit_bvh_blocks_per_cu(k);
    }
    *out = d;
    return PT_OK;
}

static int flush_pending(pt_device_s* d);

static int stream_wait(pt_device_s* d);

extern "C" int pt_device_destroy(pt_device_t d)
{
    int rc = use_device(d);
    if (rc) return rc;
    rc = flush_pending(d);
    (void)stream_wait(d);
    if (d->live_buffers != 0)
        return fail(PT_ERR_INVALID, "%d buffer(s) of this device are still alive", d->live_buffers);
    destroy_device_objects(d);
    return rc;
}

extern "C" int pt_device_info(pt_device_t d, int kind, char out[128])
{
    if (!d || !out) return fail(PT_ERR_INVALID, "null argument");
    out[0] = 0;
    switch (kind) {
    case PT_INFO_NAME:
    case PT_INFO_BOARD:
        if (d->prop.name[0]) snprintf(out, 128, "%s", d->prop.name);
        else snprintf(out, 128, "AMD Instinct (%.*s)", 96, d->prop.gcnArchName);
        break;
    case PT_INFO_VENDOR: snprintf(out, 128, "Advanced Micro Devices, Inc."); break;
    case PT_INFO_VERSION: {
        int rt = 0;
        hipRuntimeGetVersion(&rt);
        snprintf(out, 128, "HIP %d %.*s", rt, 96, d->prop.gcnArchName);
        break;
    }
    default: return fail(PT_ERR_INVALID, "unknown info kind %d", kind);
    }
    return PT_OK;
}

extern "C" uint64_t pt_device_max_alloc(pt_device_t d) { return d ? (uint64_t)d->prop.totalGlobalMem : 0; }
extern "C" uint64_t pt_device_mem_size(pt_device_t d) { return d ? (uint64_t)d->prop.totalGlobalMem : 0; }
extern "C" uint64_t pt_device_used_memory(pt_device_t d) { return d ? d->used : 0; }
extern "C" uint64_t pt_device_peak_memory(pt_device_t d) { return d ? d->peak : 0; }
extern "C" uint64_t pt_device_workspace_memory(pt_device_t d) { return d ? d->workspace : 0; }
extern "C" int pt_device_num_cus(pt_device_t d) { return d ? d->prop.multiProcessorCount : 0; }
// ... 71 lines not shown
    HIP_TRY(hipStreamWaitEvent(d->stream, (hipEvent_t)hip_event, 0));
    d->main_dirty = true;
    return PT_OK;
}

extern "C" int pt_sync(pt_device_t d)
{
    int rc = use_device(d);
    if (rc) return rc;
    if (d->pending.active && (d->pending.tris->exposed || d->pending.mats->exposed || d->pending.fb->exposed) &&
        (rc = flush_pending(d)))
        return rc;
    if ((rc = stream_wait(d))) return rc;
    return check_traversal(d);
}

extern "C" int pt_flush(pt_device_t d)
{
    int rc = use_device(d);
    if (rc) return rc;
    return flush_pending(d);
}

static int free_ring(pt_device_s* d)
{
    int rc = stream_wait(d);
    if (rc) return rc;
    ws_free(d, d->ring);
    d->ring_slot_bytes = 0;
    return PT_OK;
}

static int alloc_ring(pt_device_s* d, size_t slot_bytes)
{
    slot_bytes = (slot_bytes + 255) & ~(size_t)255;
    hipError_t e = ws_malloc(d, d->ring, PT_RING_SLOTS * slot_bytes);
    if (e != hipSuccess) return fail(PT_ERR_OOM, "radiance staging ring (%d x %zu bytes) allocation failed: %s", PT_RING_SLOTS, slot_bytes, hipGetErrorString(e));
    d->ring_slot_bytes = slot_bytes;
    return PT_OK;
}

extern "C" int pt_device_reserve_staging(pt_device_t d, size_t bytes)
{
    int rc = use_device(d);
    if (rc) return rc;
    const size_t slot = bytes ? (bytes + PT_RING_SLOTS - 1) / PT_RING_SLOTS : PT_DEFAULT_SLOT_BYTES;
    if (slot < 12) return fail(PT_ERR_INVALID, "a staging slot holds at least one 12-byte sample");
    if ((rc = flush_pending(d))) return rc;
    if (d->ring && ((slot + 255) & ~(size_t)255) == d->ring_slot_bytes) return PT_OK;
    if (d->ring && (rc = free_ring(d))) return rc;
    return alloc_ring(d, slot);
}

extern "C" int pt_device_set_option(pt_device_t d, int option, int64_t value)
{
    int rc = use_device(d);
    if (rc) return rc;
    switch (option) {
    case PT_OPT_BATCH_FRAMES:
        rc = flush_pending(d);
        d->opt_batch = value ? 1 : 0;
        return rc;
    case PT_OPT_CHUNK_FRAMES:
        if (value < 0) return fail(PT_ERR_INVALID, "chunk frames must be >= 0");
        d->opt_chunk = value;
        return PT_OK;
    case PT_OPT_PROFILE_RETURN_TIME:
        d->opt_profile = value ? 1 : 0;
        return PT_OK;
    case PT_OPT_QUAD_FILTER:
        if (value < 0 || value > 4) return fail(PT_ERR_INVALID, "quad filter must be 0 (auto), 1..3 (independent triangles) or 4 (packed shared u)");
        d->opt_quads = value;
        return PT_OK;
    case PT_OPT_ACCEL:
        if (value < 0 || value > 2) return fail(PT_ERR_INVALID, "accel must be 0 (auto), 1 (brute force) or 2 (BVH)");
        d->opt_accel = value;
        return PT_OK;
    case PT_OPT_BVH_TALLY:
        d->opt_tally = value ? 1 : 0;
        return PT_OK;
    case PT_OPT_PRIMARY_MASKS:
        d->opt_pmask = value ? 1 : 0;
        return PT_OK;
    case PT_OPT_BVH_STACK_LIMIT:
        if (value < 1 || value > 64) return fail(PT_ERR_INVALID, "the LBVH stack limit must be 1..64");
        d->opt_bvh_stack = value;
        return PT_OK;
    case PT_OPT_RENDER_LANES:
        if (value < 1 || value > 2) return fail(PT_ERR_INVALID, "render lanes must be 1 or 2");
        rc = enter_stream(d);
        d->opt_lanes = value;
        return rc;
    case PT_OPT_CHECKPOINT:
        d->opt_carry = value ? 1 : 0;
        return PT_OK;
    case PT_OPT_RESERVED_3:
        if (value != 0 && value != 1) return fail(PT_ERR_INVALID, "option 3 took 0 or 1");
        return PT_OK;
    default: return fail(PT_ERR_INVALID, "unknown option %d", option);
    }
}

extern "C" int64_t pt_device_get_option(pt_device_t d, int option)
{
    if (!d) return -1;
    switch (option) {
    case PT_OPT_BATCH_FRAMES: return d->opt_batch;
    case PT_OPT_CHUNK_FRAMES: return d->opt_chunk;
    case PT_OPT_PROFILE_RETURN_TIME: return d->opt_profile;
    case PT_OPT_QUAD_FILTER: return d->opt_quads;
    case PT_OPT_ACCEL: return d->opt_accel;
    case PT_OPT_BVH_TALLY: return d->opt_tally;
    case PT_OPT_PRIMARY_MASKS: return d->opt_pmask;
    case PT_OPT_BVH_STACK_LIMIT: return d->opt_bvh_stack;
    case PT_OPT_RENDER_LANES: return d->opt_lanes;
    case PT_OPT_CHECKPOINT: return d->opt_carry;
    case PT_OPT_BVH_BUILD_COUNT: return (int64_t)d->bvh_builds;
    case PT_OPT_RESERVED_3: return 0;
    default: return -1;
    }
}

extern "C" int pt_buffer_alloc(pt_device_t d, size_t bytes, pt_buffer_t* out)
{
    if (!out) return fail(PT_ERR_INVALID, "out == NULL");
    *out = nullptr;
    int rc = use_device(d);
    if (rc) return rc;
    pt_buffer_s* b = new (std::nothrow) pt_buffer_s();
    if (!b) return fail(PT_ERR_OOM, "host allocation failed");
    memset(static_cast<void*>(b), 0, sizeof *b);
    b->dev = d;
    b->bytes = bytes;
    b->owned = true;
    if (bytes) {
        hipError_t e = hipMalloc(&b->dptr, bytes);
        if (e != hipSuccess) {
            delete b;
            (void)hipGetLastError();
            return fail(PT_ERR_OOM, "hipMalloc(%zu) failed: %s (used %llu bytes)", bytes, hipGetErrorString(e),
                        (unsigned long long)d->used);
        }
    }
    d->used += bytes;
    d->peak = std::max(d->peak, d->used);
    d->live_buffers++;
    *out = b;
    return PT_OK;
}

extern "C" int pt_buffer_wrap(pt_device_t d, void* device_ptr, size_t bytes, pt_buffer_t* out)
{
    if (!out) return fail(PT_ERR_INVALID, "out == NULL");
    *out = nullptr;
    int rc = use_device(d);
    if (rc) return rc;
    if (!device_ptr && bytes) return fail(PT_ERR_INVALID, "null device pointer");
    pt_buffer_s* b = new (std::nothrow) pt_buffer_s();
    if (!b) return fail(PT_ERR_OOM, "host allocation failed");
    memset(static_cast<void*>(b), 0, sizeof *b);
    b->dev = d;
    b->dptr = device_ptr;
    b->bytes = bytes;
    b->owned = false;
    d->live_buffers++;
    *out = b;
    return PT_OK;
}

extern "C" int pt_buffer_free(pt_buffer_t b)
{
    if (!b) return fail(PT_ERR_INVALID, "null buffer handle");
    pt_device_s* d = b->dev;
    int rc = use_device(d);
    if (rc) return rc;
    if (d->pending.active && (d->pending.tris == b || d->pending.mats == b || d->pending.fb == b)) rc = flush_pending(d);
    (void)stream_wait(d);
    if (d->prep_src == b) d->prep_src = nullptr;
    if (b->staging) hipHostFree(b->staging);
    if (b->owned) {
        if (b->dptr) hipFree(b->dptr);
        d->used -= b->bytes;
    }
    d->live_buffers--;
    delete b;
    return rc;
}

extern "C" size_t pt_buffer_size(pt_buffer_t b) { return b ? b->bytes : 0; }
extern "C" void* pt_buffer_address(pt_buffer_t b) { return b ? b->dptr : nullptr; }

extern "C" void* pt_buffer_device_ptr(pt_buffer_t b)
{
    if (!b) return nullptr;
    if (!b->exposed) {
        b->exposed = true;
// ... 471 lines not shown

struct PtSearch {
    PtSearchMode mode;
    const PtFilterTable* ft;
    int ntri;
    int driver_blocks;
    bool wide;
};

static int prepare_search(pt_device_s* d, const pt_buffer_s* tris, int ntri, const float* eye, PtSearch& s)
{
    s = PtSearch();
    s.ft = &d->scene_filter;
    if (ntri == 0) return PT_OK;
    const bool use_bvh = ntri >= 2 && (d->opt_accel == 2 || (d->opt_accel == 0 && ntri >= PT_BVH_AUTO_MIN));
    if (!use_bvh && ntri >= (1 << 26))
        return fail(PT_ERR_INVALID, "the brute-force search packs a triangle index in 26 bits: use PT_OPT_ACCEL 0 or 2 for %d triangles", ntri);
    if (use_bvh && ntri >= (1 << 25))
        return fail(PT_ERR_INVALID, "the LBVH search packs a record index (2 x triangles) in 26 bits: %d triangles are too many", ntri);
    int rc;
    if ((rc = ensure_prep(d, tris, ntri))) return rc;
    if (use_bvh && (rc = ensure_bvh(d, tris, ntri))) return rc;
    PtFilterTable& ft = use_bvh ? d->big_filter : d->scene_filter;
    const PtCamera ref = reference_camera();
    const float* anchor = eye ? eye : ft.anchor_valid ? ft.anchor : ref.eye;
    if ((rc = use_bvh ? ensure_anchor(d, ft, d->bigtab, d->nbig, anchor) : ensure_anchor(d, ft, d->prep, d->prep_ntri, anchor))) return rc;
    s.mode = { use_bvh, d->prep_det_bounded, (d->opt_quads == 0 || d->opt_quads == 4) ? ft.quads : 0 };
    s.ft = &ft;
    s.ntri = ntri;
    s.driver_blocks = use_bvh ? d->prop.multiProcessorCount * d->query_bvh_blocks_per_cu : 0;
    s.wide = use_bvh && eye && eye_is_far(d, eye);
    return PT_OK;
}

static void search_fields(const pt_device_s* d, const PtSearch& s, PtTraceParams& t)
{
    const PtFilterTable& ft = *s.ft;
    t.tris = d->prep;
    t.ntri = s.ntri;
    t.quad_delta1 = ft.delta1; t.ray_radius = ft.ray_radius;
    t.p1tab = ft.p1tab; t.p1_lo = ft.p1_lo; t.p1_hi = ft.p1_hi;
    memcpy(t.cam.eye, ft.anchor, sizeof t.cam.eye);
    t.bvh = d->bvh; t.bvh_records = (int32_t)d->bvh_records; t.grid = d->bvh_grid;
    t.bigtab = d->bigtab; t.bigidx = d->bigidx; t.nbig = s.mode.bvh ? d->nbig : 0;
    t.bvh_flags = d->trav_dev; t.bvh_stack_limit = (int32_t)d->opt_bvh_stack;
}

static int plan_chunks(pt_device_s* d, int frame_count, uint32_t npix, int& nchunks, int& chunk)
{
    int rc;
    const uint64_t frame_bytes = (uint64_t)npix * 12;
    if (!d->ring || d->ring_slot_bytes < frame_bytes) {
        if (d->ring && (rc = free_ring(d))) return rc;
        if ((rc = alloc_ring(d, (size_t)std::max<uint64_t>(frame_bytes, PT_DEFAULT_SLOT_BYTES)))) return rc;
    }
    uint64_t slot_frames = std::min<uint64_t>(d->ring_slot_bytes / frame_bytes, 16383);
    if (d->opt_chunk > 0) slot_frames = std::min<uint64_t>(slot_frames, (uint64_t)d->opt_chunk);
    nchunks = (int)(((uint64_t)frame_count + slot_frames - 1) / slot_frames);
    chunk = (frame_count + nchunks - 1) / nchunks;
    return PT_OK;
}

static int refresh_pmask(pt_device_s* d, const pt_render_params& rp, const PtCamera& cam, uint32_t npix, bool& make)
{
    int rc;
    const int32_t g[7] = { rp.width, rp.height, rp.stripe_rows, rp.n_ranks, rp.rank, (int32_t)npix, rp.num_triangles };
    make = !d->pmask_key.valid || d->pmask_key.scene_gen != d->scene_gen || memcmp(d->pmask_key.g, g, sizeof g) != 0 ||
           memcmp(&d->pmask_key.cam, &cam, sizeof cam) != 0;
    if (!make) return PT_OK;
    if ((rc = stream_enqueue(d))) return rc;
    d->pmask_key.valid = false;
    if (d->pmask.bytes < (size_t)npix * sizeof(uint2)) {
        HIP_TRY(hipStreamSynchronize(d->stream));
        ws_free(d, d->pmask);
        hipError_t e = ws_malloc(d, d->pmask, (size_t)npix * sizeof(uint2));
        if (e != hipSuccess) return fail(PT_ERR_OOM, "primary-mask allocation (%zu bytes) failed: %s", (size_t)npix * sizeof(uint2), hipGetErrorString(e));
    }
    d->pmask_key.scene_gen = d->scene_gen;
    memcpy(d->pmask_key.g, g, sizeof g);
    d->pmask_key.cam = cam;
    return PT_OK;
}

static bool pmask_footprint_holds(int width, int height)
{
    return (double)width * width + (double)height * height <= 7626.0 * 7626.0;
}

static int choose_batch(const pt_device_s* d, bool use_bvh, uint32_t npix, int chunk, uint32_t& batch, uint32_t& bpf, int& blocks)
{
    const int wg_waves = PT_TRACE_THREADS / 64;
    blocks = d->prop.multiProcessorCount * (use_bvh ? d->bvh_blocks_per_cu : d->blocks_per_cu);
    const uint64_t resident_waves = (uint64_t)blocks * wg_waves;
    const uint64_t chunk_samples = (uint64_t)npix * (uint64_t)chunk;
    batch = PT_TRACE_BATCH;
    while (batch > 128u && chunk_samples / batch < 64u * resident_waves) batch >>= 1;
    bpf = (npix + batch - 1) / batch;
    if ((uint64_t)bpf * (uint64_t)chunk + PT_QUEUE_SHARDS > 0xffffffffull) return fail(PT_ERR_INVALID, "chunk too large");
    const uint64_t blocks_needed = ((uint64_t)bpf * (uint64_t)chunk + wg_waves - 1) / wg_waves;
    if ((uint64_t)blocks > blocks_needed) blocks = (int)blocks_needed;
    return PT_OK;
}

static void image_geometry(PtTraceParams& t, int width, int height, int stripe_rows, int n_ranks, int rank, uint32_t npix)
{
    t.width = width; t.height = height;
    t.inv_width = 1.0f / (float)width;
    t.inv_height = 1.0f / (float)height;
    t.aspect = (float)width / (float)height;
    t.stripe_rows = stripe_rows; t.n_ranks = n_ranks; t.rank = rank;
    t.npix_local = npix;
}

static PtTraceParams trace_params(const pt_device_s* d, const pt_buffer_s* mats, const pt_buffer_s* stats, const pt_render_params& rp,
                                  const PtCamera& cam, uint32_t npix, const PtSearch& search, bool use_pmask, int chunk, uint32_t batch, uint32_t bpf)
{
    PtTraceParams tp;
    memset(&tp, 0, sizeof tp);
    search_fields(d, search, tp);
    tp.mats = (const PtRawMaterial*)mats->dptr;
    tp.stats = stats ? (unsigned long long*)stats->dptr : nullptr;
    image_geometry(tp, rp.width, rp.height, rp.stripe_rows, rp.n_ranks, rp.rank, npix);
    tp.max_bounces = rp.max_bounces; tp.nmat = rp.num_materials;
    tp.batches_per_frame = bpf; tp.batch = batch;
    tp.pmask = use_pmask ? d->pmask.p : nullptr;
    tp.slot_frames = (uint32_t)chunk;
    tp.ring_magic = (uint32_t)(0x100000000ull / (2u * (uint32_t)chunk)) + 1u;
    tp.rad = d->ring;
    tp.rad1 = reinterpret_cast<float*>(reinterpret_cast<char*>(d->ring.p) + d->ring_slot_bytes);
    tp.rad1_off = (uint64_t)PT_RING_SLOTS * d->ring_slot_bytes <= 0x100000000ull ? (uint32_t)d->ring_slot_bytes : 0u;
    tp.cam = cam;
    return tp;
}

static int ensure_carry(pt_device_s* d, int blocks)
{
    const int wg_waves = PT_TRACE_THREADS / 64;
    const size_t waves = (size_t)d->prop.multiProcessorCount * 8 * wg_waves;
    if ((size_t)blocks * wg_waves > waves) return fail(PT_ERR_INVALID, "grid larger than the checkpoint regions");
    for (int k = 0; k < 2; ++k)
        if (!d->carry[k]) {
            static_assert(PT_CARRY_HIT_STRIDE_DW >= PT_CARRY_STRIDE_DW, "a checkpoint region holds either kernel's records");
            hipError_t e = ws_malloc(d, d->carry[k], waves * PT_CARRY_HIT_STRIDE_DW * sizeof(uint32_t));
            if (e != hipSuccess) return fail(PT_ERR_OOM, "checkpoint buffer allocation failed: %s", hipGetErrorString(e));
        }
    return PT_OK;
}

static int render_part(pt_device_s* d, pt_buffer_s* tris, pt_buffer_s* mats, pt_buffer_s* fb, const pt_render_params& rp, const PtCamera& cam,
                       uint32_t npix, pt_buffer_s* stats, pt_event_s* ev_start, pt_event_s* ev_stop)
{
    int rc;
    PtSearch search;
    if ((rc = prepare_search(d, tris, rp.num_triangles, cam.eye, search))) return rc;
    const bool use_bvh = search.mode.bvh;
    if (!use_bvh && rp.num_triangles <= PT_LDS_TRI_MAX && rp.max_bounces > PT_PACKED_BOUNCE_MAX)
        return fail(PT_ERR_INVALID, "max_bounces above %d on a scene of at most %d triangles without the LBVH (a parked path packs its bounce count in 8 bits)",
                    PT_PACKED_BOUNCE_MAX, PT_LDS_TRI_MAX);
    int nchunks, chunk;
    if ((rc = plan_chunks(d, rp.frame_count, npix, nchunks, chunk))) return rc;
    const bool want_pmask = d->opt_pmask && search.mode.quads == 3 && !use_bvh && rp.num_triangles <= 64 && search.mode.det_bounded;
    const bool use_pmask = want_pmask && pmask_footprint_holds(rp.width, rp.height);
    if (want_pmask && !use_pmask) d->pmask_key.valid = false;
    bool make_pmask = false;
    if (use_pmask && (rc = refresh_pmask(d, rp, cam, npix, make_pmask))) return rc;
    if (d->counters_dirty) {
        if ((rc = stream_enqueue(d))) return rc;
        HIP_TRY(hipMemsetAsync(d->counters, 0, WS_COUNTERS, d->stream));
        d->counters_dirty = false;
    }
    uint32_t batch, bpf;
    int blocks;
    if ((rc = choose_batch(d, use_bvh, npix, chunk, batch, bpf, blocks))) return rc;
    PtTraceParams tp = trace_params(d, mats, stats, rp, cam, npix, search, use_pmask, chunk, batch, bpf);
    if (make_pmask) {
        HIP_TRY(ptk_primary_masks(tp, d->stream));
        d->pmask_key.valid = true;
    }
    const bool carry = d->opt_carry != 0 && nchunks > 1;
    int ln = d->opt_lanes == 2 ? (int)(d->render_seq++ & 1u) : 0;
    hipStream_t st = d->lane[ln];
    if (carry && (rc = ensure_carry(d, blocks))) return rc;
    const int wg_waves = PT_TRACE_THREADS / 64;

    if (d->main_dirty || d->external) {
        HIP_TRY(hipEventRecord(d->ev_fork, d->stream));
        HIP_TRY(hipStreamWaitEvent(d->lane[0], d->ev_fork, 0));
        HIP_TRY(hipStreamWaitEvent(d->lane[1], d->ev_fork, 0));
        d->main_dirty = false;
    }
    d->lanes_busy = true;
    d->counters_dirty = true;
    if (ev_start) HIP_TRY(hipEventRecord(ev_start->start, st));
    tp.ring_phase = (uint32_t)((d->chunk_seq & 1u) ? chunk : 0);
    tp.carry = carry ? d->carry[ln].p : nullptr;
    unsigned int* const drain_counter = d->counters + (size_t)(PT_QUEUE_COUNTERS - 1 - ln) * PT_QUEUE_STRIDE;
    unsigned int* prev_counter = nullptr;
    int prev_slot = 0, prev_f0 = 0, prev_nf = 0;
    hipEvent_t pstop;
    bool chained = false;
    auto fold = [&](int slot, int f0, int nf, unsigned int* reset, unsigned int* reset2) -> int {
        const bool last = f0 + nf >= rp.frame_count || !carry, last_two = f0 + nf + chunk >= rp.frame_count;
        if ((!chained || !carry) && d->fold_recorded[ln ^ 1]) HIP_TRY(hipStreamWaitEvent(st, d->ev_fold[ln ^ 1], 0));
        chained = true;
        PtFoldParams fp;
        fp.rad = slot ? tp.rad1 : tp.rad;
        fp.fb = (float4*)fb->dptr;
        fp.npix_local = npix;
        fp.frame_begin = rp.frame_begin + f0;
        fp.frame_count = nf;
        fp.reset_counter = reset;
        fp.reset_counter2 = reset2;
        int r = prof_begin(d, PT_PROF_FOLD, st, &pstop);
        if (r) return r;
        HIP_TRY(ptk_fold(fp, st));
        if ((r = prof_end(st, pstop))) return r;
        if (last_two) {
            HIP_TRY(hipEventRecord(d->ev_slot[slot], st));
            d->slot_recorded[slot] = true;
        }
        if (last) {
            HIP_TRY(hipEventRecord(d->ev_fold[ln], st));
            d->fold_recorded[ln] = true;
            d->last_fold_lane = ln;
        }
        return PT_OK;
    };
    auto trace = [&](int f0, int nf, unsigned int* counter, bool carry_in, bool carry_out) -> int {
        tp.batch_counter = counter;
        tp.frame_begin = rp.frame_begin + f0;
        tp.frame_count = nf;
        tp.chunk_f0 = (uint32_t)f0;
        tp.carry_in_waves = carry_in ? (uint32_t)(blocks * wg_waves) : 0u;
        tp.carry_out = carry_out ? 1u : 0u;
        tp.total_batches = (uint32_t)((uint64_t)bpf * (uint64_t)nf);
        int r = prof_begin(d, PT_PROF_TRACE, st, &pstop);
        if (r) return r;
        HIP_TRY(ptk_trace(tp, blocks, search.mode, d->opt_tally != 0 && stats != nullptr, search.wide, st));
        return prof_end(st, pstop);
    };
    for (int c = 0; c < nchunks; ++c) {
        const int f0 = c * chunk;
        const int nf = std::min(chunk, rp.frame_count - f0);
        const uint64_t seq = d->chunk_seq++;
        const int slot = (int)(seq & 1u);
        unsigned int* counter = d->counters + (size_t)(seq % (PT_QUEUE_COUNTERS - 2)) * PT_QUEUE_STRIDE;
        if (!carry && d->opt_lanes == 2 && c > 0) {
            ln ^= 1;
            st = d->lane[ln];
        }
        if (c < 2 && d->slot_recorded[slot]) HIP_TRY(hipStreamWaitEvent(st, d->ev_slot[slot], 0));
        if ((rc = trace(f0, nf, counter, carry && c > 0, carry))) return rc;
        if (!carry) {
            if ((rc = fold(slot, f0, nf, counter, nullptr))) return rc;
        } else {
            if (c > 0 && (rc = fold(prev_slot, prev_f0, prev_nf, prev_counter, nullptr))) return rc;
            prev_slot = slot; prev_f0 = f0; prev_nf = nf; prev_counter = counter;
// ... 798 lines not shown
    if (!framebuffer || !rgb_i32) return fail(PT_ERR_INVALID, "null buffer handle");
    if (framebuffer->dev != d || rgb_i32->dev != d) return fail(PT_ERR_INVALID, "buffer belongs to another device");
    if (num_pixels * sizeof(float4) > framebuffer->bytes) return fail(PT_ERR_RANGE, "framebuffer too small");
    if (num_pixels * 3 * sizeof(int32_t) > rgb_i32->bytes) return fail(PT_ERR_RANGE, "rgb buffer too small");
    if ((rc = enter_stream(d)) || (rc = event_begin(d, ev))) return rc;
    HIP_TRY(ptk_tonemap_ppm((const float4*)framebuffer->dptr, (int32_t*)rgb_i32->dptr, num_pixels, d->stream));
    rgb_i32->version++;
    return event_end(d, ev);
}

extern "C" int pt_profile_enable(pt_device_t d, int on)
{
    int rc = use_device(d);
    if (rc) return rc;
    d->prof_on = on != 0;
    return PT_OK;
}

extern "C" int pt_profile_reset(pt_device_t d)
{
    int rc = use_device(d);
    if (rc) return rc;
    if ((rc = enter_stream(d)) || (rc = stream_wait(d))) return rc;
    for (int k = 0; k < PT_PROF_KINDS; ++k) d->prof_used[k] = 0;
    return PT_OK;
}

extern "C" int pt_profile_query(pt_device_t d, int kind, double* total_ms, uint64_t* launches)
{
    int rc = use_device(d);
    if (rc) return rc;
    if (kind < 0 || kind >= PT_PROF_KINDS || !total_ms || !launches) return fail(PT_ERR_INVALID, "bad profile query");
    if ((rc = enter_stream(d)) || (rc = stream_wait(d))) return rc;
    double sum = 0.0;
    for (size_t i = 0; i < d->prof_used[kind]; ++i) {
        float ms = 0.f;
        HIP_TRY(hipEventElapsedTime(&ms, d->prof_pairs[kind][i].first, d->prof_pairs[kind][i].second));
        sum += ms;
    }
    *total_ms = sum;
    *launches = d->prof_used[kind];
    return check_traversal(d);
}

extern "C" int pt_bvh_snapshot(pt_device_t d, pt_bvh_info* info, void* records, size_t record_capacity, int32_t* big_indices)
{
    static_assert(sizeof(pt_bvh_info) == 64, "pt_bvh_info layout");
    static_assert(PT_BVH_SNAPSHOT_BIG_MAX == PT_BVH_BIG_MAX, "the header's bound is the builder's");
    int rc = use_device(d);
    if (rc) return rc;
    if (!info) return fail(PT_ERR_INVALID, "pt_bvh_snapshot: info is null");
    if ((rc = flush_pending(d)) || (rc = stream_wait(d))) return rc;
    if (!d->bvh_valid || !d->bvh) return fail(PT_ERR_INVALID, "no LBVH stands for the prepared scene");
    memset(info, 0, sizeof *info);
    info->records = (uint32_t)d->bvh_records;
    info->num_big = d->nbig;
    info->num_triangles = d->prep_ntri;
    for (int a = 0; a < 3; ++a) { info->grid_min[a] = d->bvh_grid.gmin[a]; info->grid_step[a] = d->bvh_grid.gstep[a]; }
    if (records) {
        if (record_capacity < d->bvh_records) return fail(PT_ERR_RANGE, "pt_bvh_snapshot: %zu records do not fit %zu", d->bvh_records, record_capacity);
        if (d->bvh_records) HIP_TRY(hipMemcpy(records, d->bvh, d->bvh_records * sizeof(PtBvh8Node), hipMemcpyDeviceToHost));
    }
    if (big_indices && d->nbig > 0) HIP_TRY(hipMemcpy(big_indices, d->bigidx, (size_t)d->nbig * sizeof(int), hipMemcpyDeviceToHost));
    return PT_OK;
}

extern "C" int pt_primary_mask_snapshot(pt_device_t d, uint32_t* num_pixels, void* masks, size_t capacity)
{
    int rc = use_device(d);
    if (rc) return rc;
    if (!num_pixels) return fail(PT_ERR_INVALID, "pt_primary_mask_snapshot: num_pixels is null");
    if ((rc = flush_pending(d)) || (rc = stream_wait(d))) return rc;
    if (!d->pmask_key.valid || d->pmask_key.scene_gen != d->scene_gen || !d->pmask.p)
        return fail(PT_ERR_INVALID, "no primary-ray masks stand for the prepared scene");
    const size_t npix = (size_t)(uint32_t)d->pmask_key.g[5];
    *num_pixels = (uint32_t)npix;
    if (masks) {
        if (capacity < npix) return fail(PT_ERR_RANGE, "pt_primary_mask_snapshot: %zu pixels do not fit %zu", npix, capacity);
        if (npix) HIP_TRY(hipMemcpy(masks, d->pmask.p, npix * sizeof(uint2), hipMemcpyDeviceToHost));
    }
    return PT_OK;
}

extern "C" int pt_profile_query_union(pt_device_t d, int kind, double* union_ms)
{
    int rc = use_device(d);
    if (rc) return rc;
    if (kind < 0 || kind >= PT_PROF_KINDS || !union_ms) return fail(PT_ERR_INVALID, "bad profile query");
    if ((rc = enter_stream(d)) || (rc = stream_wait(d))) return rc;
    const size_t n = d->prof_used[kind];
    std::vector<std::pair<double, double>> iv(n);
    for (size_t i = 0; i < n; ++i) {
        float a = 0.f, b = 0.f;
        if (i) HIP_TRY(hipEventElapsedTime(&a, d->prof_pairs[kind][0].first, d->prof_pairs[kind][i].first));
        HIP_TRY(hipEventElapsedTime(&b, d->prof_pairs[kind][0].first, d->prof_pairs[kind][i].second));
        iv[i] = { (double)a, (double)b };
    }
    std::sort(iv.begin(), iv.end());
    double total = 0.0, end = -1.0e300;
    for (auto& x : iv) {
        if (x.second <= end) continue;
        total += x.second - std::max(x.first, end);
        end = x.second;
    }
    *union_ms = total;
    return PT_OK;
}

static const char* base_name(const char* path)
{
    const char* b = path;
    for (const char* p = path; *p; ++p)
        if (*p == '/' || *p == '\\') b = p + 1;
    return b;
}

extern "C" int pt_kernel_get(pt_device_t d, const char* file_name, const char* func_name, pt_kernel_t* out)
{
    if (!out) return fail(PT_ERR_INVALID, "out == NULL");
    *out = nullptr;
    if (!d || !file_name || !func_name) return fail(PT_ERR_INVALID, "null argument");
    std::string base = base_name(file_name);
    size_t dot = base.rfind('.');
    if (dot != std::string::npos) base.erase(dot);
    for (int i = 0; i < KERNEL_COUNT; ++i)
        if (base == d->kernels[i].file && strcmp(func_name, d->kernels[i].func) == 0) {
            *out = &d->kernels[i];
            return PT_OK;
        }
    return fail(PT_ERR_NOT_FOUND, "no native kernel registered for (%s, %s)", file_name, func_name);
}

static int launch_generate_colors(pt_device_s* d, const pt_launch_arg* a, int nargs, long long n, pt_event_s* ev, float* ms_out)
{
    if (nargs != 4 || !a[0].is_buffer || !a[1].is_buffer || !a[2].is_buffer || a[3].is_buffer || a[3].size != 16)
        return fail(PT_ERR_ARGS, "GenerateColors expects (buffer, buffer, buffer, int4)");
    pt_buffer_s *t = a[0].buffer, *m = a[1].buffer, *fb = a[2].buffer;
    if (!t || !m || !fb) return fail(PT_ERR_ARGS, "GenerateColors: null buffer argument");
    int32_t c[4];
    memcpy(c, a[3].data, 16);
    if (c[0] < 1 || c[1] < 1 || c[2] < 0) return fail(PT_ERR_ARGS, "GenerateColors: invalid cRes {%d,%d,%d}", c[0], c[1], c[2]);
    long long npix = std::min<long long>(n, (long long)c[0] * c[1]);
    if (npix <= 0) return PT_OK;
    if (npix > 0xffffffffLL) return fail(PT_ERR_ARGS, "too many work-items");
    if (m->bytes < sizeof(PtRawMaterial)) return fail(PT_ERR_RANGE, "material buffer too small");

    const bool observable = !t->owned || !m->owned || !fb->owned || t->exposed || m->exposed || fb->exposed;
    bool immediate = !d->opt_batch || ev || d->opt_profile || observable;
    PendingFrames& p = d->pending;
    if (p.active && !(p.tris == t && p.mats == m && p.fb == fb && p.width == c[0] && p.height == c[1] &&
                      p.pixel_count == (uint32_t)npix && p.z_begin + p.z_count == c[2] && !immediate)) {
        int rc = flush_pending(d);
        if (rc) return rc;
    }
    if (!immediate) {
        if ((size_t)36 * sizeof(PtRawTriangle) > t->bytes) return fail(PT_ERR_RANGE, "triangle buffer smaller than 36 triangles");
        if ((size_t)npix * sizeof(float4) > fb->bytes) return fail(PT_ERR_RANGE, "framebuffer smaller than the launch");
        if (t->dev != d || m->dev != d || fb->dev != d) return fail(PT_ERR_INVALID, "buffer belongs to another device");
        if (p.active) {
            p.z_count++;
        } else {
            p.active = true;
            p.tris = t; p.mats = m; p.fb = fb;
            p.width = c[0]; p.height = c[1];
            p.z_begin = c[2]; p.z_count = 1;
            p.pixel_count = (uint32_t)npix;
// ... 125 lines not shown
```

### oclpathtracer_amd/shim.py

```python
from __future__ import annotations

import ctypes
import os

_HERE = os.path.dirname(os.path.abspath(__file__))
LIB_PATH = os.environ.get("PT_SHIM_LIB") or os.path.join(_HERE, "libptshim.so")

PT_OK = 0
PT_ERR_INVALID, PT_ERR_NO_DEVICE, PT_ERR_OOM, PT_ERR_HIP, PT_ERR_NOT_FOUND, PT_ERR_ARGS, PT_ERR_RANGE, PT_ERR_TRAVERSAL = range(1, 9)
PT_INFO_NAME, PT_INFO_BOARD, PT_INFO_VENDOR, PT_INFO_VERSION = range(4)
PT_OPT_BATCH_FRAMES, PT_OPT_CHUNK_FRAMES, PT_OPT_PROFILE_RETURN_TIME = 0, 1, 2
PT_OPT_QUAD_FILTER, PT_OPT_ACCEL, PT_OPT_BVH_TALLY, PT_OPT_PRIMARY_MASKS, PT_OPT_BVH_STACK_LIMIT, PT_OPT_RENDER_LANES, PT_OPT_CHECKPOINT, PT_OPT_BVH_BUILD_COUNT = 4, 5, 6, 7, 8, 9, 10, 11
PT_SHIM_ABI_VERSION = 2
PT_MAX_ARG_SIZE = 64
PT_MAX_ARG_COUNT = 64
PT_STAT_SAMPLES, PT_STAT_RAYS, PT_STAT_WORDS = 0, 1, 16
PT_STAT_BVH_NODES, PT_STAT_BVH_TRIS, PT_STAT_BVH_STEPS, PT_STAT_BVH_TRI_STEPS, PT_STAT_BVH_MAX_STACK, PT_STAT_CARRIED, PT_STAT_BVH_GRAZING = 2, 3, 4, 5, 6, 7, 8
PT_PROF_TRACE, PT_PROF_FOLD = 0, 1
PT_STREAM_LEGACY = 1
PT_QUERY_CLOSEST, PT_QUERY_OCCLUDED = 0, 1

_c = ctypes
_H = _c.c_void_p


class LaunchArg(_c.Structure):

    _fields_ = [
        ("is_buffer", _c.c_int32),
        ("read_only", _c.c_int32),
        ("size", _c.c_uint64),
        ("buffer", _H),
        ("data", _c.c_ubyte * PT_MAX_ARG_SIZE),
    ]


class RenderParams(_c.Structure):

    _fields_ = [
        ("width", _c.c_int32), ("height", _c.c_int32),
        ("frame_begin", _c.c_int32), ("frame_count", _c.c_int32),
        ("max_bounces", _c.c_int32), ("num_triangles", _c.c_int32), ("num_materials", _c.c_int32),
        ("stripe_rows", _c.c_int32), ("n_ranks", _c.c_int32), ("rank", _c.c_int32),
        ("reserved", _c.c_int32 * 6),
    ]


class Camera(_c.Structure):

    _fields_ = [
        ("eye", _c.c_float * 3), ("center", _c.c_float * 3), ("up", _c.c_float * 3),
        ("fov_y_deg", _c.c_float),
        ("reserved", _c.c_int32 * 6),
    ]


class Ray(_c.Structure):

    _fields_ = [("origin", _c.c_float * 3), ("tmax", _c.c_float), ("dir", _c.c_float * 3), ("reserved", _c.c_int32)]


class Hit(_c.Structure):

    _fields_ = [
        ("t", _c.c_float), ("tri", _c.c_int32), ("u", _c.c_float), ("v", _c.c_float),
        ("p", _c.c_float * 3), ("material", _c.c_int32),
        ("n", _c.c_float * 3), ("reserved", _c.c_int32),
    ]


class AoParams(_c.Structure):

    _fields_ = [
        ("width", _c.c_int32), ("height", _c.c_int32),
        ("frame_begin", _c.c_int32), ("frame_count", _c.c_int32),
        ("num_triangles", _c.c_int32), ("rays_per_sample", _c.c_int32),
        ("radius", _c.c_float), ("miss_value", _c.c_float),
        ("stripe_rows", _c.c_int32), ("n_ranks", _c.c_int32), ("rank", _c.c_int32),
        ("reserved", _c.c_int32 * 5),
    ]


class DirectParams(_c.Structure):

    _fields_ = [
        ("width", _c.c_int32), ("height", _c.c_int32),
        ("frame_begin", _c.c_int32), ("frame_count", _c.c_int32),
        ("num_triangles", _c.c_int32), ("num_materials", _c.c_int32), ("num_lights", _c.c_int32),
        ("light_samples", _c.c_int32),
        ("stripe_rows", _c.c_int32), ("n_ranks", _c.c_int32), ("rank", _c.c_int32),
        ("reserved", _c.c_int32 * 5),
    ]


class IndirectParams(_c.Structure):
# ... 67 lines not shown
    "pt_device_count": (_c.c_int, []),
    "pt_device_create": (_c.c_int, [_c.c_int, _c.POINTER(_H)]),
    "pt_device_destroy": (_c.c_int, [_H]),
    "pt_device_info": (_c.c_int, [_H, _c.c_int, _c.c_char_p]),
    "pt_device_max_alloc": (_c.c_uint64, [_H]),
    "pt_device_mem_size": (_c.c_uint64, [_H]),
    "pt_device_used_memory": (_c.c_uint64, [_H]),
    "pt_device_peak_memory": (_c.c_uint64, [_H]),
    "pt_device_workspace_memory": (_c.c_uint64, [_H]),
    "pt_device_reserve_staging": (_c.c_int, [_H, _c.c_size_t]),
    "pt_device_num_cus": (_c.c_int, [_H]),
    "pt_device_set_stream": (_c.c_int, [_H, _c.c_void_p]),
    "pt_device_get_stream": (_c.c_void_p, [_H]),
    "pt_device_wait_stream": (_c.c_int, [_H, _c.c_void_p]),
    "pt_device_wait_hip_event": (_c.c_int, [_H, _c.c_void_p]),
    "pt_event_wait_on": (_c.c_int, [_H, _c.c_void_p]),
    "pt_sync": (_c.c_int, [_H]),
    "pt_flush": (_c.c_int, [_H]),
    "pt_device_set_option": (_c.c_int, [_H, _c.c_int, _c.c_int64]),
    "pt_device_get_option": (_c.c_int64, [_H, _c.c_int]),
    "pt_buffer_alloc": (_c.c_int, [_H, _c.c_size_t, _c.POINTER(_H)]),
    "pt_buffer_wrap": (_c.c_int, [_H, _c.c_void_p, _c.c_size_t, _c.POINTER(_H)]),
    "pt_buffer_free": (_c.c_int, [_H]),
    "pt_buffer_size": (_c.c_size_t, [_H]),
    "pt_buffer_device_ptr": (_c.c_void_p, [_H]),
    "pt_buffer_address": (_c.c_void_p, [_H]),
    "pt_buffer_write": (_c.c_int, [_H, _c.c_void_p, _c.c_size_t, _c.c_size_t, _H]),
    "pt_buffer_read": (_c.c_int, [_H, _c.c_void_p, _c.c_size_t, _c.c_size_t, _H]),
    "pt_buffer_copy": (_c.c_int, [_H, _H, _c.c_size_t, _c.c_size_t, _c.c_size_t, _H]),
    "pt_buffer_map": (_c.c_void_p, [_H, _c.c_size_t, _c.c_int]),
    "pt_buffer_unmap": (_c.c_int, [_H, _c.c_void_p]),
    "pt_host_alloc": (_c.c_int, [_c.c_size_t, _c.POINTER(_c.c_void_p)]),
    "pt_host_free": (_c.c_int, [_c.c_void_p]),
    "pt_event_create": (_c.c_int, [_H, _c.POINTER(_H)]),
    "pt_event_destroy": (_c.c_int, [_H]),
    "pt_event_wait": (_c.c_int, [_H]),
    "pt_event_is_complete": (_c.c_int, [_H]),
    "pt_event_elapsed_ns": (_c.c_int, [_H, _c.POINTER(_c.c_uint64)]),
    "pt_kernel_get": (_c.c_int, [_H, _c.c_char_p, _c.c_char_p, _c.POINTER(_H)]),
    "pt_launch_2d": (_c.c_int, [_H, _H, _c.POINTER(LaunchArg), _c.c_int, _c.c_int, _c.c_int, _c.c_int, _c.c_int, _H,
                                _c.POINTER(_c.c_float)]),
    "pt_local_rows": (_c.c_int, [_c.c_int, _c.c_int, _c.c_int, _c.c_int]),
    "pt_render_frames": (_c.c_int, [_H, _H, _H, _H, _c.POINTER(RenderParams), _H, _H]),
    "pt_camera_reference": (None, [_c.POINTER(Camera)]),
    "pt_camera_derive": (_c.c_int, [_c.POINTER(Camera), _c.POINTER(_c.c_float)]),
    "pt_render_frames_camera": (_c.c_int, [_H, _H, _H, _H, _c.POINTER(RenderParams), _c.POINTER(Camera), _H, _H]),
    "pt_intersect_rays": (_c.c_int, [_H, _H, _c.c_int, _H, _H, _c.c_size_t, _c.c_int, _H]),
    "pt_camera_rays": (_c.c_int, [_H, _c.POINTER(Camera), _c.c_int, _c.c_int, _c.c_int, _H, _H]),
    "pt_occluded_rays": (_c.c_int, [_H, _H, _c.c_int, _H, _H, _c.c_size_t, _H]),
    "pt_render_ao": (_c.c_int, [_H, _H, _H, _H, _c.POINTER(AoParams), _c.POINTER(Camera), _H]),
    "pt_render_direct": (_c.c_int, [_H, _H, _H, _H, _H, _H, _c.POINTER(DirectParams), _c.POINTER(Camera), _H]),
    "pt_render_indirect": (_c.c_int, [_H, _H, _H, _H, _H, _H, _c.POINTER(IndirectParams), _c.POINTER(Camera), _H]),
    "pt_light_counts": (_c.c_int, [_H, _H, _c.c_int, _c.c_int, _H, _H]),
    "pt_render_indirect_mis": (_c.c_int, [_H, _H, _H, _H, _H, _H, _H, _c.POINTER(IndirectParams), _c.POINTER(Camera), _H]),
    "pt_light_table_bytes": (_c.c_size_t, [_c.c_int]),
    "pt_light_table": (_c.c_int, [_H, _H, _c.c_int, _H, _c.c_int, _H, _c.c_int, _H, _H, _H]),
    "pt_render_direct_power": (_c.c_int, [_H, _H, _H, _H, _H, _H, _H, _H, _c.POINTER(DirectParams), _c.POINTER(Camera), _H]),
    "pt_render_indirect_power": (_c.c_int, [_H, _H, _H, _H, _c.c_int, _H, _H, _H, _H, _H, _c.POINTER(IndirectParams), _c.POINTER(Camera), _H]),
    "pt_render_indirect_rr": (_c.c_int, [_H, _H, _H, _H, _c.c_int, _H, _H, _H, _H, _H, _c.POINTER(IndirectParams), _c.POINTER(Roulette),
                                         _c.POINTER(Camera), _H]),
    "pt_sample_moments": (_c.c_int, [_H, _H, _H, _c.c_uint32, _c.c_int32, _c.c_int, _H]),
    "pt_moments_summary_bytes": (_c.c_size_t, [_c.c_uint32]),
    "pt_moments_resolve": (_c.c_int, [_H, _H, _c.c_uint32, _H, _H, _H]),
    "pt_adaptive_list_bytes": (_c.c_size_t, [_c.c_uint32]),
    "pt_adaptive_select": (_c.c_int, [_H, _H, _c.c_uint32, _c.POINTER(AdaptiveRule), _H, _H]),
    "pt_render_indirect_pixels": (_c.c_int, [_H, _H, _H, _H, _c.c_int, _H, _H, _H, _H, _H, _H, _c.c_uint32, _c.POINTER(IndirectParams),
                                             _c.POINTER(Roulette), _c.POINTER(Camera), _H]),
    "pt_render_direct_ris": (_c.c_int, [_H, _H, _H, _H, _H, _H, _H, _H, _c.POINTER(DirectParams), _c.POINTER(Ris), _c.POINTER(Camera), _H]),
    "pt_render_indirect_ris": (_c.c_int, [_H, _H, _H, _H, _c.c_int, _H, _H, _H, _H, _H, _c.POINTER(IndirectParams), _c.POINTER(Roulette),
                                          _c.POINTER(Ris), _c.POINTER(Camera), _H]),
    "pt_render_indirect_pixels_ris": (_c.c_int, [_H, _H, _H, _H, _c.c_int, _H, _H, _H, _H, _H, _H, _c.c_uint32, _c.POINTER(IndirectParams),
                                                 _c.POINTER(Roulette), _c.POINTER(Ris), _c.POINTER(Camera), _H]),
    "pt_sample_moments_pixels": (_c.c_int, [_H, _H, _H, _H, _c.c_uint32, _c.c_int32, _H]),
    "pt_env_table_bytes": (_c.c_size_t, [_c.c_int]),
    "pt_env_table": (_c.c_int, [_H, _H, _c.c_int, _H, _H]),
    "pt_render_direct_env": (_c.c_int, [_H, _H, _H, _H, _H, _H, _H, _H, _H, _H, _c.POINTER(DirectParams), _c.POINTER(Environment),
                                        _c.POINTER(Camera), _H]),
    "pt_render_indirect_env": (_c.c_int, [_H, _H, _H, _H, _H, _H, _H, _H, _H, _H, _H, _c.POINTER(IndirectParams), _c.POINTER(Roulette),
                                          _c.POINTER(Environment), _c.POINTER(Camera), _H]),
    "pt_profile_enable": (_c.c_int, [_H, _c.c_int]),
    "pt_profile_query": (_c.c_int, [_H, _c.c_int, _c.POINTER(_c.c_double), _c.POINTER(_c.c_uint64)]),
    "pt_bvh_snapshot": (_c.c_int, [_H, _c.POINTER(BvhInfo), _c.c_void_p, _c.c_size_t, _c.c_void_p]),
    "pt_primary_mask_snapshot": (_c.c_int, [_H, _c.POINTER(_c.c_uint32), _c.c_void_p, _c.c_size_t]),
    "pt_profile_query_union": (_c.c_int, [_H, _c.c_int, _c.POINTER(_c.c_double)]),
    "pt_profile_reset": (_c.c_int, [_H]),
    "pt_assemble_stripes": (_c.c_int, [_H, _H, _H, _c.c_int, _c.c_int, _c.c_int, _c.c_int, _c.c_int, _H]),
    "pt_assemble_stripes_on": (_c.c_int, [_H, _H, _H, _c.c_int, _c.c_int, _c.c_int, _c.c_int, _c.c_int, _c.c_void_p]),
    "pt_tonemap_ppm": (_c.c_int, [_H, _H, _H, _c.c_size_t, _H]),
}


class ShimError(RuntimeError):
    def __init__(self, code: int, message: str):
        super().__init__("pt_shim error %d: %s" % (code, message))
        self.code = code


_lib = None


def load():
    global _lib
    if _lib is None:
        if not os.path.exists(LIB_PATH):
            raise ShimError(PT_ERR_NO_DEVICE, "libptshim.so is not built (run __graft_entry__.build()); "
                                              "there is no CPU fallback for the hot path")
        lib = ctypes.CDLL(LIB_PATH)
        for name, (res, args) in SIGNATURES.items():
            fn = getattr(lib, name)
            fn.restype = res
            fn.argtypes = args
        if lib.pt_abi_version() != PT_SHIM_ABI_VERSION:
            raise ShimError(PT_ERR_INVALID, "libptshim.so speaks ABI version %d, this binding %d: rebuild (__graft_entry__.build())"
                            % (lib.pt_abi_version(), PT_SHIM_ABI_VERSION))
        _lib = lib
    return _lib


def check(rc: int) -> None:
    if rc != PT_OK:
        raise ShimError(rc, load().pt_last_error().decode("utf-8", "replace"))
```

Measured before the change: 9368 Msamples/s.

## Add precomputed secondary-ray triangle masks keyed by origin tile and direction cell

Adds a per-scene table, built on the device, that maps each source triangle, a tile of positions on it and a cube-map direction cell to a conservative 64-bit mask of triangles a bounce ray could hit. Secondary rays in the small-scene quad path look up this mask and call the masked intersector instead of the two-pass full test, to skip triangle tests that cannot hit. In exchange it adds a classification step and extra global loads per bounce, and a sizeable table built on scene change with a host sync. Correctness rests on the conservative double-precision bounds in the mask generator.

```diff
diff --git a/include/pt_shim.h b/include/pt_shim.h
--- a/include/pt_shim.h
+++ b/include/pt_shim.h
@@ -73,7 +73,8 @@
     PT_OPT_BVH_STACK_LIMIT = 8,
     PT_OPT_RENDER_LANES = 9,
     PT_OPT_CHECKPOINT = 10,
-    PT_OPT_BVH_BUILD_COUNT = 11
+    PT_OPT_BVH_BUILD_COUNT = 11,
+    PT_OPT_SECONDARY_MASKS = 12
 };
 int pt_device_set_option(pt_device_t dev, int option, int64_t value);
 int64_t pt_device_get_option(pt_device_t dev, int option);
@@ -342,6 +343,8 @@
 
 int pt_primary_mask_snapshot(pt_device_t dev, uint32_t* num_pixels, void* masks, size_t capacity);
 
+int pt_secondary_mask_snapshot(pt_device_t dev, uint32_t info[4], void* masks, size_t capacity);
+
 int pt_assemble_stripes(pt_device_t dev, pt_buffer_t gathered, pt_buffer_t image, int width,
                         int height, int stripe_rows, int n_ranks, int slab_rows, pt_event_t ev);
 
diff --git a/oclpathtracer_amd/csrc/pt_kernels.h b/oclpathtracer_amd/csrc/pt_kernels.h
--- a/oclpathtracer_amd/csrc/pt_kernels.h
+++ b/oclpathtracer_amd/csrc/pt_kernels.h
@@ -93,6 +93,7 @@
     uint32_t carry_in_waves;
     uint32_t carry_out;
     PtCamera cam;
+    const uint2* smask;
 };
 #define PT_QUEUE_SHARDS 8
 #define PT_QUEUE_SHARD_WORDS 1056
@@ -132,6 +133,7 @@
 #define PT_P1_STRIDE 24
 static inline size_t ptk_p1tab_floats(int ntri) { return (size_t)((ntri / 2 + 1) / 2) * PT_P1_STRIDE; }
 hipError_t ptk_primary_masks(const PtTraceParams& p, hipStream_t s);
+hipError_t ptk_secondary_masks(const PtPrepTriangle* tris, int ntri, uint2* table, hipStream_t s);
 struct PtSearchMode {
     bool bvh;
     bool det_bounded;
diff --git a/oclpathtracer_amd/csrc/pt_kernels.hip b/oclpathtracer_amd/csrc/pt_kernels.hip
--- a/oclpathtracer_amd/csrc/pt_kernels.hip
+++ b/oclpathtracer_amd/csrc/pt_kernels.hip
@@ -1,6 +1,7 @@
 #include "pt_kernels.h"
 
 #include "pt_device_math.h"
+#include "pt_secmask.h"
 
 #include <type_traits>
 
@@ -218,6 +219,15 @@
         m[c] |= (keep ? 1u : 0u) << (nc - 1 - (j & 31));
     }
     P.out[lp] = make_uint2(m[0], m[1]);
+}
+
+__global__ void pt_secondary_mask_kernel(const PtPrepTriangle* tris, int ntri, uint2* table)
+{
+    const unsigned e = blockIdx.x * blockDim.x + threadIdx.x;
+    if (e < (unsigned)ntri) reinterpret_cast<PtSmTri*>(table)[e] = pt_sm_tri_record(tris[e].p1, tris[e].e1, tris[e].e2);
+    if (e >= (unsigned)ntri * PT_SM_TRI_ENTRIES) return;
+    const PtSmMask m = pt_sm_entry(reinterpret_cast<const float*>(tris), ntri, e);
+    table[PT_SM_HEAD_ENTRIES + e] = make_uint2(m.x, m.y);
 }
 
 struct PtTriRec { float p1x, p1y, p1z, e1x, e1y, e1z, e2x, e2y, e2z; };
@@ -634,7 +644,7 @@
 }
 
 template <bool DET_BOUNDED, int LDS_TABLE>
-PTK_DEV unsigned pt_intersect_primary(pt_const_f32p T, const PtPrepTriangle* tris, int ntri, const f3& o, const f3& d, bool alive,
+PTK_DEV unsigned pt_intersect_masked(pt_const_f32p T, const PtPrepTriangle* tris, int ntri, const f3& o, const f3& d, bool alive,
                                       float& tmax, float& hu, float& hv, int& hidx, uint2 pm, PtTail tl, unsigned lane,
                                       unsigned long long* vstat = nullptr)
 {
@@ -1229,6 +1239,9 @@
 #ifndef PT_TRACE_UNIT_DIR
 #define PT_TRACE_UNIT_DIR 1
 #endif
+#ifndef PT_TRACE_SECONDARY_MASKS
+#define PT_TRACE_SECONDARY_MASKS 1
+#endif
 template <bool DET_BOUNDED, int LDS_TABLE, int QUADS>
 PTK_DEV void pt_trace_body(const PtTraceParams& P)
 {
@@ -1304,10 +1317,56 @@
         int hidx = -1;
         unsigned p2steps = 0;
         n_rays += (unsigned)__popcll(alive);
+        bool masked = false;
+        uint2 pm = make_uint2(0u, 0u);
+        if (QUADS == 3 && DET_BOUNDED && alive != 0ull) {
+            if (primary && P.pmask != nullptr) {
+                pm = P.pmask[pix0 + lane];
+                masked = true;
+            } else if (LDS_TABLE == 1 && PT_TRACE_SECONDARY_MASKS && !fresh) {
+                const pt_kargs_p KS = pt_kargs();
+                const uint2* const sm = KS->smask;
+                const int nt = KS->ntri;
+                if (sm != nullptr) {
+#if PT_STAMPS
+                    unsigned long long ta = 0, tb = 0;
+                    PT_STAMP(ta);
+#endif
+                    const PtSmMask ones = pt_sm_all_ones(nt);
+                    pm = make_uint2(ones.x, ones.y);
+                    if (PT_ON(alive)) {
+                        const char* const base = reinterpret_cast<const char*>(sm);
+                        const unsigned k = (unsigned)h.hidx < (unsigned)(nt - 1) ? (unsigned)h.hidx : (unsigned)(nt - 1);
+                        const float4 ra = *reinterpret_cast<const float4*>(base + (size_t)(k * 48u));
+                        const float4 rb = *reinterpret_cast<const float4*>(base + (size_t)(k * 48u + 16u));
+                        const float4 rn = *reinterpret_cast<const float4*>(base + (size_t)(k * 48u + 32u));
+                        const float A[4] = { ra.x, ra.y, ra.z, ra.w }, B[4] = { rb.x, rb.y, rb.z, rb.w }, N[4] = { rn.x, rn.y, rn.z, rn.w };
+                        unsigned entry;
+                        const bool covered = pt_sm_classify(A, B, N, s.o.x, s.o.y, s.o.z, s.d.x, s.d.y, s.d.z, k, &entry);
+                        const uint2 v = *reinterpret_cast<const uint2*>(base + (size_t)(entry * 8u + (unsigned)(PT_SM_HEAD_ENTRIES * 8)));
+                        if (covered) pm = v;
+#if PT_VALIDATE_FILTER
+                        if (P.stats) {
+                            const pt_lanes unc = PT_LANES(!covered);
+                            if (lane == (unsigned)__builtin_ctzll(alive)) {
+                                atomicAdd(&P.stats[10], (unsigned long long)__popcll(alive));
+                                atomicAdd(&P.stats[11], (unsigned long long)__popcll(unc & alive));
+                            }
+                        }
+#endif
+                    }
+                    masked = true;
+#if PT_STAMPS
+                    PT_STAMP(tb);
+                    c_p1 += tb - ta;
+#endif
+                }
+            }
+        }
         if (alive == 0ull) {
-        } else if (QUADS == 3 && DET_BOUNDED && primary && P.pmask != nullptr)
-            p2steps = pt_intersect_primary<DET_BOUNDED, LDS_TABLE>(T, P.tris, ntri, s.o, s.d, PT_ON(alive), tmax, hu, hv, hidx, P.pmask[pix0 + lane], tl, lane,
-                                                                   PT_VALIDATE_FILTER && P.stats ? P.stats + 2 : nullptr);
+        } else if (masked)
+            p2steps = pt_intersect_masked<DET_BOUNDED, LDS_TABLE>(T, P.tris, ntri, s.o, s.d, PT_ON(alive), tmax, hu, hv, hidx, pm, tl, lane,
+                                                                  PT_VALIDATE_FILTER && P.stats ? P.stats + 2 : nullptr);
         else
             p2steps = pt_intersect_two_pass<DET_BOUNDED, LDS_TABLE, QUADS, PT_TRACE_UNIT_DIR != 0>(T, P.tris, ntri, s.o, s.d, PT_ON(alive), tmax, hu, hv, hidx,
                                                                                           P.quad_delta1, P.ray_radius,
@@ -3884,6 +3943,14 @@
     return hipGetLastError();
 }
 
+hipError_t ptk_secondary_masks(const PtPrepTriangle* tris, int ntri, uint2* table, hipStream_t s)
+{
+    if (!table || ntri <= 0 || ntri > PT_SM_TRI_MAX) return hipErrorInvalidValue;
+    const unsigned n = (unsigned)ntri * PT_SM_TRI_ENTRIES;
+    hipLaunchKernelGGL(pt_secondary_mask_kernel, dim3((n + 255u) / 256u), dim3(256), 0, s, tris, ntri, table);
+    return hipGetLastError();
+}
+
 hipError_t ptk_trace(const PtTraceParams& p, int num_blocks, PtSearchMode m, bool tally, bool wide, hipStream_t s)
 {
     const bool q3 = m.quads == 3;
diff --git a/oclpathtracer_amd/csrc/pt_secmask.h b/oclpathtracer_amd/csrc/pt_secmask.h
--- /dev/null
+++ b/oclpathtracer_amd/csrc/pt_secmask.h
@@ -0,0 +1,218 @@
+#pragma once
+
+#include <math.h>
+#include <stdint.h>
+
+#if defined(__HIPCC__)
+#define PT_SM_HD __host__ __device__ static inline
+#else
+#define PT_SM_HD static inline
+#endif
+
+#ifndef PT_SM_T
+#define PT_SM_T 12
+#endif
+#ifndef PT_SM_C
+#define PT_SM_C 8
+#endif
+#ifndef PT_SM_SO
+#define PT_SM_SO 2
+#endif
+#ifndef PT_SM_SD
+#define PT_SM_SD 4
+#endif
+#define PT_SM_GUARD (1.0 / 64.0)
+#define PT_SM_DIRS (6 * PT_SM_C * PT_SM_C)
+#define PT_SM_TRI_ENTRIES (PT_SM_T * PT_SM_T * PT_SM_DIRS)
+#define PT_SM_TRI_MAX 64
+struct PtSmTri { float A[4], B[4], N[4]; };
+#define PT_SM_HEAD_ENTRIES (PT_SM_TRI_MAX * sizeof(PtSmTri) / 8)
+#define PT_SM_TABLE_BYTES(ntri) ((PT_SM_HEAD_ENTRIES + (size_t)(ntri) * PT_SM_TRI_ENTRIES) * 8)
+
+struct PtSmMask { unsigned x, y; };
+
+PT_SM_HD float pt_sm_form(const float* F, float ox, float oy, float oz)
+{
+    return __builtin_fmaf(F[2], oz, __builtin_fmaf(F[1], oy, __builtin_fmaf(F[0], ox, F[3])));
+}
+
+PT_SM_HD bool pt_sm_classify(const float* A, const float* B, const float* N, float ox, float oy, float oz, float dx, float dy, float dz,
+                             unsigned k, unsigned* entry)
+{
+    const float tu = pt_sm_form(A, ox, oy, oz), tv = pt_sm_form(B, ox, oy, oz), th = pt_sm_form(N, ox, oy, oz);
+    const float dd = __builtin_fmaf(dz, dz, __builtin_fmaf(dy, dy, dx * dx));
+    const bool covered = (tu >= 0.0f) & (tu < (float)PT_SM_T) & (tv >= 0.0f) & (tv < (float)PT_SM_T) & (__builtin_fabsf(th) <= 1.0f) &
+                         (dd >= 0.999f) & (dd <= 1.001f);
+    const float ax = __builtin_fabsf(dx), ay = __builtin_fabsf(dy), az = __builtin_fabsf(dz);
+    const bool mx = (ax >= ay) & (ax >= az), my = ay >= az;
+    const unsigned m = mx ? 0u : my ? 1u : 2u;
+    const float dm = mx ? dx : my ? dy : dz;
+    const float da = mx ? dy : my ? dz : dx;
+    const float db = mx ? dz : my ? dx : dy;
+#if defined(__HIP_DEVICE_COMPILE__)
+    const float r = __builtin_amdgcn_rcpf(__builtin_fabsf(dm));
+#else
+    const float r = 1.0f / __builtin_fabsf(dm);
+#endif
+    const float ca = covered ? __builtin_fmaf(da * r, 0.5f * PT_SM_C, 0.5f * PT_SM_C) : 0.0f;
+    const float cb = covered ? __builtin_fmaf(db * r, 0.5f * PT_SM_C, 0.5f * PT_SM_C) : 0.0f;
+    const float ca_c = __builtin_fminf(__builtin_fmaxf(ca, 0.0f), (float)(PT_SM_C - 1));
+    const float cb_c = __builtin_fminf(__builtin_fmaxf(cb, 0.0f), (float)(PT_SM_C - 1));
+    const unsigned ia = (unsigned)(int)ca_c, ib = (unsigned)(int)cb_c;
+    const unsigned iu = (unsigned)(int)(covered ? tu : 0.0f), iv = (unsigned)(int)(covered ? tv : 0.0f);
+    const unsigned face = 2u * m + (dm < 0.0f ? 1u : 0u);
+    *entry = ((k * PT_SM_T + iu) * PT_SM_T + iv) * PT_SM_DIRS + (face * PT_SM_C + ia) * PT_SM_C + ib;
+    return covered;
+}
+
+struct PtSmV3 { double x, y, z; };
+PT_SM_HD PtSmV3 pt_sm_v(double x, double y, double z) { PtSmV3 r = { x, y, z }; return r; }
+PT_SM_HD PtSmV3 pt_sm_vf(const float* p) { return pt_sm_v((double)p[0], (double)p[1], (double)p[2]); }
+PT_SM_HD PtSmV3 pt_sm_cross(PtSmV3 a, PtSmV3 b) { return pt_sm_v(a.y * b.z - a.z * b.y, a.z * b.x - a.x * b.z, a.x * b.y - a.y * b.x); }
+PT_SM_HD double pt_sm_dot(PtSmV3 a, PtSmV3 b) { return a.x * b.x + a.y * b.y + a.z * b.z; }
+PT_SM_HD PtSmV3 pt_sm_sub(PtSmV3 a, PtSmV3 b) { return pt_sm_v(a.x - b.x, a.y - b.y, a.z - b.z); }
+PT_SM_HD PtSmV3 pt_sm_axpy(double s, PtSmV3 a, PtSmV3 b) { return pt_sm_v(s * a.x + b.x, s * a.y + b.y, s * a.z + b.z); }
+PT_SM_HD double pt_sm_n1(PtSmV3 a) { return fabs(a.x) + fabs(a.y) + fabs(a.z); }
+PT_SM_HD double pt_sm_absdot(PtSmV3 r, PtSmV3 a) { return r.x * fabs(a.x) + r.y * fabs(a.y) + r.z * fabs(a.z); }
+
+#define PT_SM_U 5.9604644775390625e-8
+
+struct PtSmGeom {
+    PtSmV3 p1, e1, e2, nh;
+    double H, du, dv, dh;
+    PtSmTri rec;
+    bool valid;
+};
+
+PT_SM_HD void pt_sm_form_make(PtSmV3 w, double c, double scale, PtSmV3 reach, PtSmV3 p1, float* F, double* E)
+{
+    F[0] = (float)(w.x * scale); F[1] = (float)(w.y * scale); F[2] = (float)(w.z * scale);
+    F[3] = (float)((c - pt_sm_dot(w, p1)) * scale);
+    *E = fabs((double)F[0]) * (fabs(p1.x) + reach.x) + fabs((double)F[1]) * (fabs(p1.y) + reach.y) + fabs((double)F[2]) * (fabs(p1.z) + reach.z) +
+         fabs((double)F[3]);
+}
+
+PT_SM_HD PtSmGeom pt_sm_geom(const float* p1, const float* e1, const float* e2)
+{
+    PtSmGeom g;
+    g.p1 = pt_sm_vf(p1); g.e1 = pt_sm_vf(e1); g.e2 = pt_sm_vf(e2);
+    const PtSmV3 n = pt_sm_cross(g.e1, g.e2);
+    const double nn = pt_sm_dot(n, n), ln = sqrt(nn);
+    g.nh = pt_sm_v(n.x / ln, n.y / ln, n.z / ln);
+    const PtSmV3 as = pt_sm_cross(g.e2, n), bs = pt_sm_cross(n, g.e1);
+    const double ext = fmax(fabs(g.p1.x) + fabs(g.e1.x) + fabs(g.e2.x), fmax(fabs(g.p1.y) + fabs(g.e1.y) + fabs(g.e2.y), fabs(g.p1.z) + fabs(g.e1.z) + fabs(g.e2.z)));
+    g.H = 0.0101 + 32.0 * PT_SM_U * ext;
+    const double G = PT_SM_GUARD, st = (double)PT_SM_T / (1.0 + 2.0 * G);
+    const PtSmV3 reach = pt_sm_v((1.0 + G) * (fabs(g.e1.x) + fabs(g.e2.x)) + g.H, (1.0 + G) * (fabs(g.e1.y) + fabs(g.e2.y)) + g.H,
+                                 (1.0 + G) * (fabs(g.e1.z) + fabs(g.e2.z)) + g.H);
+    double Eu, Ev, Eh;
+    pt_sm_form_make(pt_sm_v(as.x / nn, as.y / nn, as.z / nn), G, st, reach, g.p1, g.rec.A, &Eu);
+    pt_sm_form_make(pt_sm_v(bs.x / nn, bs.y / nn, bs.z / nn), G, st, reach, g.p1, g.rec.B, &Ev);
+    pt_sm_form_make(g.nh, 0.0, 1.0 / g.H, reach, g.p1, g.rec.N, &Eh);
+    g.du = 8.0 * PT_SM_U * Eu; g.dv = 8.0 * PT_SM_U * Ev; g.dh = 8.0 * PT_SM_U * Eh;
+    bool ok = nn > 0.0 && g.du <= 0.25 && g.dv <= 0.25 && g.dh <= 0.25;
+    ok = ok && 0.0101 * sqrt(pt_sm_dot(as, as)) / nn <= G && 0.0101 * sqrt(pt_sm_dot(bs, bs)) / nn <= G;
+    for (int i = 0; i < 4; ++i)
+        ok = ok && fabs((double)g.rec.A[i]) < 1e30 && fabs((double)g.rec.B[i]) < 1e30 && fabs((double)g.rec.N[i]) < 1e30;
+    g.valid = ok;
+    if (!ok)
+        for (int i = 0; i < 4; ++i) g.rec.A[i] = g.rec.B[i] = g.rec.N[i] = __builtin_nanf("");
+    return g;
+}
+
+PT_SM_HD PtSmTri pt_sm_tri_record(const float* p1, const float* e1, const float* e2) { return pt_sm_geom(p1, e1, e2).rec; }
+
+PT_SM_HD PtSmMask pt_sm_all_ones(int ntri)
+{
+    PtSmMask m;
+    const int n0 = ntri < 32 ? ntri : 32, n1 = ntri - 32 < 0 ? 0 : ntri - 32 > 32 ? 32 : ntri - 32;
+    m.x = n0 == 32 ? ~0u : (1u << n0) - 1u;
+    m.y = n1 == 32 ? ~0u : (1u << n1) - 1u;
+    return m;
+}
+
+PT_SM_HD void pt_sm_ratio_range(int i, double* lo, double* hi)
+{
+    const double dc = 1e-4;
+    *lo = fmax(-1.0, ((double)i - dc) * (2.0 / PT_SM_C) - 1.0);
+    *hi = fmin(1.0, ((double)i + 1.0 + dc) * (2.0 / PT_SM_C) - 1.0);
+}
+PT_SM_HD double pt_sm_absmin(double lo, double hi) { return lo > 0.0 ? lo : hi < 0.0 ? -hi : 0.0; }
+PT_SM_HD double pt_sm_absmax(double lo, double hi) { return fmax(fabs(lo), fabs(hi)); }
+PT_SM_HD void pt_sm_set(PtSmV3* v, unsigned axis, double x) { if (axis == 0u) v->x = x; else if (axis == 1u) v->y = x; else v->z = x; }
+
+PT_SM_HD bool pt_sm_keep(const PtSmGeom& g, PtSmV3 oc, double ru, double rv, double Hr, PtSmV3 dc, PtSmV3 rd, const float* tj)
+{
+    const double INF = 1.001, ABS = 2e-24, RHO = 32.0 * PT_SM_U;
+    const PtSmV3 q1 = pt_sm_vf(tj), f1 = pt_sm_vf(tj + 3), f2 = pt_sm_vf(tj + 6);
+    const PtSmV3 tc = pt_sm_sub(oc, q1);
+    const double f1n = pt_sm_n1(f1), f2n = pt_sm_n1(f2);
+    const double tv1 = pt_sm_n1(tc) + ru * pt_sm_n1(g.e1) + rv * pt_sm_n1(g.e2) + 3.0 * Hr;
+    const PtSmV3 Kd = pt_sm_cross(f2, f1);
+    const double det_hi = pt_sm_dot(dc, Kd) + ((pt_sm_absdot(rd, Kd) + RHO * f1n * f2n) * INF + ABS);
+    if (det_hi < 0.999e-8) return false;
+    const PtSmV3 Gt = pt_sm_cross(f1, f2);
+    const double tn_c = pt_sm_dot(tc, Gt);
+    const double tn_r = (ru * fabs(pt_sm_dot(g.e1, Gt)) + rv * fabs(pt_sm_dot(g.e2, Gt)) + Hr * fabs(pt_sm_dot(g.nh, Gt)) + RHO * tv1 * f1n * f2n) * INF + ABS;
+    if (tn_c + tn_r <= 0.0) return false;
+    const PtSmV3 Ku = pt_sm_cross(f2, tc), Du = pt_sm_cross(dc, f2);
+    const PtSmV3 x1 = pt_sm_cross(f2, g.e1), x2 = pt_sm_cross(f2, g.e2), x3 = pt_sm_cross(f2, g.nh);
+    const double un_c = pt_sm_dot(dc, Ku);
+    const double un_r = (pt_sm_absdot(rd, Ku) + ru * fabs(pt_sm_dot(g.e1, Du)) + rv * fabs(pt_sm_dot(g.e2, Du)) + Hr * fabs(pt_sm_dot(g.nh, Du)) +
+                         ru * pt_sm_absdot(rd, x1) + rv * pt_sm_absdot(rd, x2) + Hr * pt_sm_absdot(rd, x3) + RHO * tv1 * f2n) * INF + ABS;
+    if (un_c + un_r < 0.0) return false;
+    const PtSmV3 Kv = pt_sm_cross(tc, f1), Dv = pt_sm_cross(f1, dc);
+    const PtSmV3 y1 = pt_sm_cross(f1, g.e1), y2 = pt_sm_cross(f1, g.e2), y3 = pt_sm_cross(f1, g.nh);
+    const double vn_c = pt_sm_dot(dc, Kv);
+    const double vn_r = (pt_sm_absdot(rd, Kv) + ru * fabs(pt_sm_dot(g.e1, Dv)) + rv * fabs(pt_sm_dot(g.e2, Dv)) + Hr * fabs(pt_sm_dot(g.nh, Dv)) +
+                         ru * pt_sm_absdot(rd, y1) + rv * pt_sm_absdot(rd, y2) + Hr * pt_sm_absdot(rd, y3) + RHO * tv1 * f1n) * INF + ABS;
+    if (vn_c + vn_r < 0.0) return false;
+    if ((un_c - un_r) + (vn_c - vn_r) > det_hi * 1.000002) return false;
+    return true;
+}
+
+PT_SM_HD PtSmMask pt_sm_entry(const float* tris, int ntri, unsigned entry)
+{
+    const unsigned k = entry / PT_SM_TRI_ENTRIES, within = entry - k * PT_SM_TRI_ENTRIES;
+    const unsigned tile = within / PT_SM_DIRS, cell = within - tile * PT_SM_DIRS;
+    const unsigned iu = tile / PT_SM_T, iv = tile - iu * PT_SM_T;
+    const unsigned face = cell / (PT_SM_C * PT_SM_C), ia = (cell / PT_SM_C) % PT_SM_C, ib = cell % PT_SM_C;
+    const float* tk = tris + 16 * k;
+    const PtSmGeom g = pt_sm_geom(tk, tk + 3, tk + 6);
+    const PtSmMask ones = pt_sm_all_ones(ntri);
+    if (!g.valid) return ones;
+    const double G = PT_SM_GUARD, su = (1.0 + 2.0 * G) / PT_SM_T, Hr = g.H * (1.0 + g.dh);
+    const unsigned m = face >> 1, a = (m + 1u) % 3u, b = (m + 2u) % 3u;
+    const double s = (face & 1u) ? -1.0 : 1.0;
+    double qa0, qa1, qb0, qb1;
+    pt_sm_ratio_range((int)ia, &qa0, &qa1);
+    pt_sm_ratio_range((int)ib, &qb0, &qb1);
+    const double tu0 = (double)iu - g.du, tuw = (1.0 + 2.0 * g.du) / PT_SM_SO, tv0 = (double)iv - g.dv, tvw = (1.0 + 2.0 * g.dv) / PT_SM_SO;
+    const double qaw = (qa1 - qa0) / PT_SM_SD, qbw = (qb1 - qb0) / PT_SM_SD;
+    PtSmMask out = { 0u, 0u };
+    for (int sd = 0; sd < PT_SM_SD * PT_SM_SD; ++sd) {
+        const double a0 = qa0 + qaw * (sd / PT_SM_SD), a1 = a0 + qaw, b0 = qb0 + qbw * (sd % PT_SM_SD), b1 = b0 + qbw;
+        const double amin = pt_sm_absmin(a0, a1), amax = pt_sm_absmax(a0, a1), bmin = pt_sm_absmin(b0, b1), bmax = pt_sm_absmax(b0, b1);
+        const double l0 = 0.9994 / sqrt(1.0 + amax * amax + bmax * bmax), l1 = 1.0006 / sqrt(1.0 + amin * amin + bmin * bmin);
+        const double a_lo = fmin(a0 * l0, a0 * l1), a_hi = fmax(a1 * l0, a1 * l1);
+        const double b_lo = fmin(b0 * l0, b0 * l1), b_hi = fmax(b1 * l0, b1 * l1);
+        PtSmV3 dc = pt_sm_v(0, 0, 0), rd = pt_sm_v(0, 0, 0);
+        pt_sm_set(&dc, m, s * 0.5 * (l0 + l1)); pt_sm_set(&rd, m, 0.5 * (l1 - l0));
+        pt_sm_set(&dc, a, 0.5 * (a_lo + a_hi)); pt_sm_set(&rd, a, 0.5 * (a_hi - a_lo));
+        pt_sm_set(&dc, b, 0.5 * (b_lo + b_hi)); pt_sm_set(&rd, b, 0.5 * (b_hi - b_lo));
+        for (int so = 0; so < PT_SM_SO * PT_SM_SO; ++so) {
+            const double uc = (tu0 + tuw * ((so / PT_SM_SO) + 0.5)) * su - G, vc = (tv0 + tvw * ((so % PT_SM_SO) + 0.5)) * su - G;
+            const double ru = 0.5 * tuw * su * (1.0 + 1e-9), rv = 0.5 * tvw * su * (1.0 + 1e-9);
+            const PtSmV3 oc = pt_sm_axpy(uc, g.e1, pt_sm_axpy(vc, g.e2, g.p1));
+            for (int j = 0; j < ntri; ++j) {
+                const int c = j >> 5;
+                const int nc = ntri - 32 * c < 32 ? ntri - 32 * c : 32;
+                const unsigned bit = 1u << (nc - 1 - (j & 31));
+                if ((c == 0 ? out.x : out.y) & bit) continue;
+                if (pt_sm_keep(g, oc, ru, rv, Hr, dc, rd, tris + 16 * j)) { if (c == 0) out.x |= bit; else out.y |= bit; }
+            }
+        }
+        if (out.x == ones.x && out.y == ones.y) break;
+    }
+    return out;
+}
diff --git a/oclpathtracer_amd/csrc/pt_shim.hip b/oclpathtracer_amd/csrc/pt_shim.hip
--- a/oclpathtracer_amd/csrc/pt_shim.hip
+++ b/oclpathtracer_amd/csrc/pt_shim.hip
@@ -15,6 +15,7 @@
 #include <vector>
 
 #include "pt_kernels.h"
+#include "pt_secmask.h"
 
 static thread_local char g_err[512] = "";
 
@@ -92,7 +93,7 @@
     uint64_t used, peak;
     int live_buffers;
     uint64_t workspace;
-    int64_t opt_batch, opt_chunk, opt_profile, opt_quads, opt_accel, opt_tally, opt_pmask, opt_bvh_stack, opt_lanes, opt_carry;
+    int64_t opt_batch, opt_chunk, opt_profile, opt_quads, opt_accel, opt_tally, opt_pmask, opt_bvh_stack, opt_lanes, opt_carry, opt_smask;
     pt_kernel_s kernels[KERNEL_COUNT];
     PendingFrames pending;
     PtWs<PtPrepTriangle> prep;
@@ -138,6 +139,8 @@
     PtWs<uint32_t> carry[2];
     PtWs<uint2> pmask;
     struct { uint64_t scene_gen; int32_t g[7]; PtCamera cam; bool valid; } pmask_key;
+    PtWs<uint2> smask;
+    struct { uint64_t scene_gen; int32_t ntri; bool valid, declined; } smask_key;
     PtWs<unsigned int> counters;
     bool counters_dirty;
     bool prof_on;
@@ -177,6 +180,10 @@
 #define PT_DEFAULT_PRIMARY_MASKS 1
 #endif
 
+#ifndef PT_DEFAULT_SECONDARY_MASKS
+#define PT_DEFAULT_SECONDARY_MASKS 1
+#endif
+
 static int g_init_count = 0;
 
 template <class T> static hipError_t ws_malloc(pt_device_s* d, PtWs<T>& w, size_t bytes)
@@ -237,6 +244,7 @@
     ws_free(d, d->bvh);
     ws_free(d, d->ring);
     ws_free(d, d->pmask);
+    ws_free(d, d->smask);
     ws_free(d, d->counters);
     ws_free(d, d->bigtab);
     ws_free(d, d->bigidx);
@@ -288,6 +296,7 @@
     d->stream = d->own_stream;
     d->opt_batch = 1;
     d->opt_pmask = PT_DEFAULT_PRIMARY_MASKS;
+    d->opt_smask = PT_DEFAULT_SECONDARY_MASKS;
     d->opt_bvh_stack = 64;
     d->opt_lanes = 2;
     d->opt_carry = 1;
@@ -525,6 +534,9 @@
     case PT_OPT_PRIMARY_MASKS:
         d->opt_pmask = value ? 1 : 0;
         return PT_OK;
+    case PT_OPT_SECONDARY_MASKS:
+        d->opt_smask = value ? 1 : 0;
+        return PT_OK;
     case PT_OPT_BVH_STACK_LIMIT:
         if (value < 1 || value > 64) return fail(PT_ERR_INVALID, "the LBVH stack limit must be 1..64");
         d->opt_bvh_stack = value;
@@ -555,6 +567,7 @@
     case PT_OPT_ACCEL: return d->opt_accel;
     case PT_OPT_BVH_TALLY: return d->opt_tally;
     case PT_OPT_PRIMARY_MASKS: return d->opt_pmask;
+    case PT_OPT_SECONDARY_MASKS: return d->opt_smask;
     case PT_OPT_BVH_STACK_LIMIT: return d->opt_bvh_stack;
     case PT_OPT_RENDER_LANES: return d->opt_lanes;
     case PT_OPT_CHECKPOINT: return d->opt_carry;
@@ -1192,6 +1205,36 @@
     return PT_OK;
 }
 
+static int refresh_smask(pt_device_s* d, int ntri)
+{
+    int rc;
+    if ((d->smask_key.valid || d->smask_key.declined) && d->smask_key.scene_gen == d->scene_gen && d->smask_key.ntri == ntri) return PT_OK;
+    if ((rc = stream_enqueue(d))) return rc;
+    d->smask_key.valid = d->smask_key.declined = false;
+    {
+        PtPrepTriangle host[PT_SM_TRI_MAX];
+        HIP_TRY(hipMemcpyAsync(host, d->prep.p, (size_t)ntri * sizeof(PtPrepTriangle), hipMemcpyDeviceToHost, d->stream));
+        HIP_TRY(hipStreamSynchronize(d->stream));
+        bool all = true;
+        for (int k = 0; k < ntri && all; ++k) all = pt_sm_geom(host[k].p1, host[k].e1, host[k].e2).valid;
+        d->smask_key.scene_gen = d->scene_gen;
+        d->smask_key.ntri = ntri;
+        d->smask_key.declined = !all;
+        if (!all) return PT_OK;
+    }
+    if (d->smask.bytes < PT_SM_TABLE_BYTES(ntri)) {
+        HIP_TRY(hipStreamSynchronize(d->stream));
+        ws_free(d, d->smask);
+        hipError_t e = ws_malloc(d, d->smask, PT_SM_TABLE_BYTES(ntri));
+        if (e != hipSuccess) return fail(PT_ERR_OOM, "secondary-mask allocation (%zu bytes) failed: %s", (size_t)PT_SM_TABLE_BYTES(ntri), hipGetErrorString(e));
+    }
+    HIP_TRY(ptk_secondary_masks(d->prep, ntri, d->smask, d->stream));
+    d->smask_key.scene_gen = d->scene_gen;
+    d->smask_key.ntri = ntri;
+    d->smask_key.valid = true;
+    return PT_OK;
+}
+
 static bool pmask_footprint_holds(int width, int height)
 {
     return (double)width * width + (double)height * height <= 7626.0 * 7626.0;
@@ -1274,6 +1317,10 @@
     if (want_pmask && !use_pmask) d->pmask_key.valid = false;
     bool make_pmask = false;
     if (use_pmask && (rc = refresh_pmask(d, rp, cam, npix, make_pmask))) return rc;
+    const bool can_smask = search.mode.quads == 3 && !use_bvh && rp.num_triangles <= PT_SM_TRI_MAX && search.mode.det_bounded;
+    const bool use_smask = can_smask && d->opt_smask;
+    if (!can_smask) d->smask_key.valid = d->smask_key.declined = false;
+    if (use_smask && (rc = refresh_smask(d, rp.num_triangles))) return rc;
     if (d->counters_dirty) {
         if ((rc = stream_enqueue(d))) return rc;
         HIP_TRY(hipMemsetAsync(d->counters, 0, WS_COUNTERS, d->stream));
@@ -1283,6 +1330,7 @@
     int blocks;
     if ((rc = choose_batch(d, use_bvh, npix, chunk, batch, bpf, blocks))) return rc;
     PtTraceParams tp = trace_params(d, mats, stats, rp, cam, npix, search, use_pmask, chunk, batch, bpf);
+    tp.smask = use_smask && d->smask_key.valid ? d->smask.p : nullptr;
     if (make_pmask) {
         HIP_TRY(ptk_primary_masks(tp, d->stream));
         d->pmask_key.valid = true;
@@ -2247,6 +2295,23 @@
     return PT_OK;
 }
 
+extern "C" int pt_secondary_mask_snapshot(pt_device_t d, uint32_t info[4], void* masks, size_t capacity)
+{
+    int rc = use_device(d);
+    if (rc) return rc;
+    if (!info) return fail(PT_ERR_INVALID, "pt_secondary_mask_snapshot: info is null");
+    if ((rc = flush_pending(d)) || (rc = stream_wait(d))) return rc;
+    if (!d->smask_key.valid || d->smask_key.scene_gen != d->scene_gen || d->smask_key.ntri != d->prep_ntri || !d->smask.p)
+        return fail(PT_ERR_INVALID, "no secondary-ray masks stand for the prepared scene");
+    const size_t n = (size_t)d->smask_key.ntri * PT_SM_TRI_ENTRIES;
+    info[0] = (uint32_t)n; info[1] = (uint32_t)d->smask_key.ntri; info[2] = PT_SM_T; info[3] = PT_SM_C;
+    if (masks) {
+        if (capacity < n) return fail(PT_ERR_RANGE, "pt_secondary_mask_snapshot: %zu entries do not fit %zu", n, capacity);
+        HIP_TRY(hipMemcpy(masks, d->smask.p + PT_SM_HEAD_ENTRIES, n * sizeof(uint2), hipMemcpyDeviceToHost));
+    }
+    return PT_OK;
+}
+
 extern "C" int pt_profile_query_union(pt_device_t d, int kind, double* union_ms)
 {
     int rc = use_device(d);
diff --git a/oclpathtracer_amd/shim.py b/oclpathtracer_amd/shim.py
--- a/oclpathtracer_amd/shim.py
+++ b/oclpathtracer_amd/shim.py
@@ -11,6 +11,7 @@
 PT_INFO_NAME, PT_INFO_BOARD, PT_INFO_VENDOR, PT_INFO_VERSION = range(4)
 PT_OPT_BATCH_FRAMES, PT_OPT_CHUNK_FRAMES, PT_OPT_PROFILE_RETURN_TIME = 0, 1, 2
 PT_OPT_QUAD_FILTER, PT_OPT_ACCEL, PT_OPT_BVH_TALLY, PT_OPT_PRIMARY_MASKS, PT_OPT_BVH_STACK_LIMIT, PT_OPT_RENDER_LANES, PT_OPT_CHECKPOINT, PT_OPT_BVH_BUILD_COUNT = 4, 5, 6, 7, 8, 9, 10, 11
+PT_OPT_SECONDARY_MASKS = 12
 PT_SHIM_ABI_VERSION = 2
 PT_MAX_ARG_SIZE = 64
 PT_MAX_ARG_COUNT = 64
@@ -244,6 +245,7 @@
     "pt_profile_query": (_c.c_int, [_H, _c.c_int, _c.POINTER(_c.c_double), _c.POINTER(_c.c_uint64)]),
     "pt_bvh_snapshot": (_c.c_int, [_H, _c.POINTER(BvhInfo), _c.c_void_p, _c.c_size_t, _c.c_void_p]),
     "pt_primary_mask_snapshot": (_c.c_int, [_H, _c.POINTER(_c.c_uint32), _c.c_void_p, _c.c_size_t]),
+    "pt_secondary_mask_snapshot": (_c.c_int, [_H, _c.POINTER(_c.c_uint32), _c.c_void_p, _c.c_size_t]),
     "pt_profile_query_union": (_c.c_int, [_H, _c.c_int, _c.POINTER(_c.c_double)]),
     "pt_profile_reset": (_c.c_int, [_H]),
     "pt_assemble_stripes": (_c.c_int, [_H, _H, _H, _c.c_int, _c.c_int, _c.c_int, _c.c_int, _c.c_int, _H]),
```

After: 9881 Msamples/s (median of 6 runs). 1.05x the previous value.
